# cslab-ntua/sparsex

Hardware: AMD Instinct MI355X
Metric: SpMV GFLOP/s (2*nnz/t, alpha=0.5, x/y resident in HBM) (higher is better)
Workload: dtype f64

## Files before the change

include/sparsex_hip.h:

```cpp
#ifndef SPARSEX_HIP_H
#define SPARSEX_HIP_H

#include <sparsex/sparsex.h>
#include <stdint.h>

#ifdef __cplusplus
extern "C" {
#endif

spx_error_t spx_hip_matvec_mult(spx_value_t alpha, const spx_matrix_t *A,
                                const spx_value_t *x_dev, spx_value_t *y_dev,
                                void *stream);
spx_error_t spx_hip_matvec_kernel(spx_value_t alpha, const spx_matrix_t *A,
                                  const spx_value_t *x_dev, spx_value_t beta,
                                  spx_value_t *y_dev, void *stream);

spx_error_t spx_hip_matmat_kernel(spx_value_t alpha, const spx_matrix_t *A, size_t nvec,
                                  const spx_value_t *X_dev, size_t ldx, spx_value_t beta,
                                  spx_value_t *Y_dev, size_t ldy, void *stream);
int spx_hip_matmat_group(const spx_matrix_t *A);

typedef struct spx_hip_vec spx_hip_vec_t;

void spx_hip_vec_touch(const spx_vector_t *v);
// ... 48 lines not shown
spx_hip_transport_t *spx_hip_transport_rccl(const void *id, int rank, int world);
void spx_hip_transport_destroy(spx_hip_transport_t *t);
int spx_hip_transport_rccl_ranks(const spx_hip_transport_t *t);

spx_error_t spx_hip_mat_dist_attach(spx_matrix_t *A, const spx_hip_transport_t *t);

#define SPX_DIST_OWNED_ROWS 0
#define SPX_DIST_GATHER_Y   1
#define SPX_DIST_HALO_X     2
#define SPX_DIST_OVERLAP    4
spx_error_t spx_hip_matvec_dist(spx_value_t alpha, const spx_matrix_t *A,
                                const spx_value_t *x_dev, spx_value_t beta,
                                spx_value_t *y_dev, int flags, void *stream);

typedef struct {
    int32_t rank, world;
    const spx_index_t *row_lo, *row_hi;
    int64_t n_send;
    const spx_index_t *send_rows;
    const size_t *send_off, *send_cnt;
    int64_t n_recv;
    const size_t *recv_off, *recv_cnt;
    int64_t n_fix_rows;
    const spx_index_t *fix_rows;
    const uint32_t *fix_ptr, *fix_pos;
    int32_t any_exchange;
} spx_hip_dist_plan_t;
spx_error_t spx_hip_mat_dist_plan(const spx_matrix_t *A, spx_hip_dist_plan_t *plan);

#define SPX_DIST_REORDER_RCM        1
#define SPX_DIST_REORDER_RCM_OWNER  2
#define SPX_DIST_PATTERN_SYMMETRIC  1
spx_error_t spx_hip_dist_reorder(const spx_index_t *rowptr, const spx_index_t *colind, spx_index_t nrows,
                                 int indexing , int world,
                                 int mode, int flags, spx_index_t *perm);

typedef struct {
    int64_t n_recv;
    const spx_index_t *recv_cols;
    const size_t *recv_off, *recv_cnt;
    int64_t n_send;
    const spx_index_t *send_rows;
    const size_t *send_off, *send_cnt;
} spx_hip_dist_halo_t;
spx_error_t spx_hip_mat_dist_halo(const spx_matrix_t *A, spx_hip_dist_halo_t *halo);

spx_error_t spx_hip_matvec_parts(spx_value_t alpha, const spx_matrix_t *A, const spx_value_t *x_dev,
                                 spx_value_t beta, spx_value_t *y_dev, int parts, void *stream, int *launched);

int spx_hip_mat_dist_rounds(const spx_matrix_t *A);
int spx_hip_mat_dist_parts(const spx_matrix_t *A);
spx_error_t spx_hip_mat_dist_round(const spx_matrix_t *A, int round, const size_t **send_off, const size_t **send_cnt,
                                   const size_t **recv_off, const size_t **recv_cnt);

typedef struct {
    int64_t nnz;
    int64_t nnz_stored;
    int64_t n_unit_elems;
    int64_t n_delta_elems;
    int64_t n_units;
    int64_t n_rowblocks;
    int64_t n_shared_rows;
    int64_t value_bytes;
    int64_t index_bytes;
    int32_t nr_partitions;
    int32_t first_partition, last_partition;
    int32_t row_lo, row_hi;
    int32_t symmetric;
    int32_t on_device;
    int32_t device;
    int32_t waves;
    int32_t sym_tiles;
    double  tune_seconds;
    double  emit_seconds;
    int32_t wave_tiles;
    int32_t sym_segments;
    int32_t quad;
    int32_t col_slices;
    int32_t unit_windows;
    int32_t unit_window_lds;
    int64_t unit_window_elems;
    int64_t unit_window_staged;
    int32_t sym_pipeline;
    int32_t reserved0;
    int64_t sym_pipeline_elems;
} spx_hip_info_t;

spx_error_t spx_hip_mat_info(const spx_matrix_t *A, spx_hip_info_t *info);

typedef struct {
    const uint32_t *tab;
    const uint32_t *xdescs;
    const void *passes;
    size_t n_rowblocks, n_descs, n_passes;
    size_t rowblocks_with_windows, rowblocks_with_units;
    uint64_t staged_doubles;
    uint64_t unit_elems, unit_elems_lds;
    uint32_t lds_doubles;
} spx_hip_xw_plan_t;
spx_error_t spx_hip_mat_unit_windows(spx_matrix_t *A, uint32_t budget, uint32_t gap, spx_hip_xw_plan_t *plan);

typedef struct {
    const void *passes;
    const uint32_t *n_sx;
    size_t n_rowblocks, n_passes;
    size_t rowblocks_with_sx;
    uint64_t sym_elems, sx_elems;
    uint64_t sym_passes, sx_passes;
} spx_hip_sx_plan_t;
spx_error_t spx_hip_mat_sym_pipeline(spx_matrix_t *A, spx_hip_sx_plan_t *plan);
#define SPX_HIP_ABI_VERSION 5
spx_error_t spx_hip_mat_info_sized(const spx_matrix_t *A, void *info, size_t size);
int spx_hip_abi_version(void);

int spx_hip_mat_host_parts(const spx_matrix_t *A);
int spx_hip_mat_host_order(const spx_matrix_t *A, int32_t *order, int cap);
int64_t spx_hip_mat_x_pieces(spx_matrix_t *A, size_t piece, uint64_t *mask, uint32_t *row0, uint32_t *n_rows, size_t cap);

typedef struct {
    const spx_value_t *values;
    const uint8_t *ctl;
    int64_t ctl_size;
    spx_index_t nnz, ncols, nrows, row_start;
    int32_t row_jumps;
    int32_t full_colind;
    long id_map[64];
    const spx_index_t *rows_info;
    const spx_value_t *dvalues;
} spx_csx_export_t;

spx_error_t spx_hip_mat_export_csx(const spx_matrix_t *A, int part,
                                   spx_csx_export_t *out);

typedef struct {
    int32_t type, delta, size, row, col;
} spx_unit_record_t;

int64_t spx_hip_mat_export_units(const spx_matrix_t *A, int part,
                                 spx_unit_record_t *recs, int64_t cap);

const char *spx_hip_mat_tune_log(const spx_matrix_t *A);

void spx_hip_xform(int from, int to, spx_index_t *row, spx_index_t *col,
                   spx_index_t nr_rows, spx_index_t nr_cols);

void spx_hip_options_reset(void);

#ifdef __cplusplus
}
#endif

#endif
```

sparsex_amd/api.py:

```python
import ctypes as C
import os

import numpy as np

SPX_SUCCESS = 0
SPX_FAILURE = -1
SPX_MAT_REORDER = 42
SPX_VEC_AS_IS = 43
SPX_VEC_TUNE = 44
SPX_INDEX_ZERO_BASED = 45
SPX_INDEX_ONE_BASED = 46

_HERE = os.path.dirname(os.path.abspath(__file__))


def lib_path():
    return os.environ.get("SPX_LIB_PATH") or os.path.join(_HERE, "lib", "libsparsex.so")


class SpxError(RuntimeError):
    pass


class VectorStruct(C.Structure):
    _fields_ = [("elements", C.POINTER(C.c_double)), ("size", C.c_size_t),
                ("alloc_type", C.c_int), ("vec_mode", C.c_int)]


class HipInfo(C.Structure):
    _fields_ = [("nnz", C.c_int64), ("nnz_stored", C.c_int64),
                ("n_unit_elems", C.c_int64), ("n_delta_elems", C.c_int64),
                ("n_units", C.c_int64), ("n_rowblocks", C.c_int64),
                ("n_shared_rows", C.c_int64), ("value_bytes", C.c_int64),
                ("index_bytes", C.c_int64), ("nr_partitions", C.c_int32),
                ("first_partition", C.c_int32), ("last_partition", C.c_int32),
                ("row_lo", C.c_int32), ("row_hi", C.c_int32),
                ("symmetric", C.c_int32), ("on_device", C.c_int32),
                ("device", C.c_int32), ("waves", C.c_int32), ("sym_tiles", C.c_int32),
                ("tune_seconds", C.c_double),
                ("emit_seconds", C.c_double), ("wave_tiles", C.c_int32), ("sym_segments", C.c_int32),
                ("quad", C.c_int32), ("col_slices", C.c_int32),
                ("unit_windows", C.c_int32), ("unit_window_lds", C.c_int32),
                ("unit_window_elems", C.c_int64), ("unit_window_staged", C.c_int64),
                ("sym_pipeline", C.c_int32), ("reserved0", C.c_int32), ("sym_pipeline_elems", C.c_int64)]


class SxPlan(C.Structure):
    _fields_ = [("passes", C.c_void_p), ("n_sx", C.POINTER(C.c_uint32)), ("n_rowblocks", C.c_size_t),
                ("n_passes", C.c_size_t), ("rowblocks_with_sx", C.c_size_t), ("sym_elems", C.c_uint64),
                ("sx_elems", C.c_uint64), ("sym_passes", C.c_uint64), ("sx_passes", C.c_uint64)]


class XwPlan(C.Structure):
    _fields_ = [("tab", C.POINTER(C.c_uint32)), ("xdescs", C.POINTER(C.c_uint32)), ("passes", C.c_void_p),
                ("n_rowblocks", C.c_size_t), ("n_descs", C.c_size_t), ("n_passes", C.c_size_t),
                ("rowblocks_with_windows", C.c_size_t), ("rowblocks_with_units", C.c_size_t),
                ("staged_doubles", C.c_uint64), ("unit_elems", C.c_uint64), ("unit_elems_lds", C.c_uint64),
                ("lds_doubles", C.c_uint32)]


class CsxExport(C.Structure):
    _fields_ = [("values", C.POINTER(C.c_double)), ("ctl", C.POINTER(C.c_uint8)),
                ("ctl_size", C.c_int64), ("nnz", C.c_int), ("ncols", C.c_int),
                ("nrows", C.c_int), ("row_start", C.c_int),
                ("row_jumps", C.c_int32), ("full_colind", C.c_int32),
                ("id_map", C.c_long * 64), ("rows_info", C.POINTER(C.c_int)),
                ("dvalues", C.POINTER(C.c_double))]


class UnitRecord(C.Structure):
    _fields_ = [("type", C.c_int32), ("delta", C.c_int32), ("size", C.c_int32),
                ("row", C.c_int32), ("col", C.c_int32)]


_lib = None


def lib():
    global _lib
    if _lib is not None:
        return _lib
    path = lib_path()
    if not os.path.exists(path):
        raise SpxError(
            "libsparsex.so is not built (%s); run `make lib` or "
            "__graft_entry__.build() -- there is no fallback path" % path)
    L = C.CDLL(path, mode=C.RTLD_GLOBAL)
    vp, i, d = C.c_void_p, C.c_int, C.c_double
    L.spx_input_load_csr.restype = vp
    L.spx_input_load_mmf.restype = vp
    L.spx_input_load_mmf.argtypes = [C.c_char_p]
    L.spx_input_destroy.argtypes = [vp]
    L.spx_mat_tune.restype = vp
    L.spx_mat_destroy.argtypes = [vp]
    L.spx_mat_get_nrows.argtypes = [vp]
    L.spx_mat_get_ncols.argtypes = [vp]
    L.spx_mat_get_nnz.argtypes = [vp]
    L.spx_mat_get_partition.restype = vp
    L.spx_mat_get_partition.argtypes = [vp]
    L.spx_partition_get_rs.restype = C.POINTER(C.c_int)
    L.spx_partition_get_rs.argtypes = [vp]
    L.spx_partition_get_re.restype = C.POINTER(C.c_int)
    L.spx_partition_get_re.argtypes = [vp]
    L.spx_partition_destroy.argtypes = [vp]
    L.spx_option_set.argtypes = [C.c_char_p, C.c_char_p]
    L.spx_option_set.restype = None
    L.spx_hip_options_reset.restype = None
    L.spx_vec_create_from_buff.restype = C.POINTER(VectorStruct)
    L.spx_vec_create_from_buff.argtypes = [C.POINTER(C.c_double), vp, C.c_size_t, vp,
                                           C.c_uint]
    L.spx_vec_destroy.argtypes = [C.POINTER(VectorStruct)]
    L.spx_vec_destroy.restype = None
    L.spx_matvec_mult.argtypes = [d, vp, C.POINTER(VectorStruct), C.POINTER(VectorStruct)]
    L.spx_matvec_kernel.argtypes = [d, vp, C.POINTER(VectorStruct), d,
                                    C.POINTER(VectorStruct)]
    L.spx_hip_matvec_mult.argtypes = [d, vp, vp, vp, vp]
    L.spx_hip_matvec_kernel.argtypes = [d, vp, vp, d, vp, vp]
    L.spx_hip_mat_info.argtypes = [vp, C.POINTER(HipInfo)]
    L.spx_hip_mat_export_csx.argtypes = [vp, i, C.POINTER(CsxExport)]
    L.spx_hip_mat_export_units.restype = C.c_int64
    L.spx_hip_mat_export_units.argtypes = [vp, i, C.POINTER(UnitRecord), C.c_int64]
    L.spx_hip_mat_tune_log.restype = C.c_char_p
    L.spx_hip_mat_tune_log.argtypes = [vp]
    L.spx_hip_vec_create.restype = vp
    L.spx_hip_vec_create.argtypes = [C.c_size_t]
    L.spx_hip_vec_destroy.argtypes = [vp]
    L.spx_hip_vec_data.restype = vp
# ... 90 lines not shown
        try:
            if beta is None:
                rc = L.spx_matvec_mult(alpha, self.handle, xv, yv)
            else:
                rc = L.spx_matvec_kernel(alpha, self.handle, xv, beta, yv)
        finally:
            L.spx_vec_destroy(xv)
            L.spx_vec_destroy(yv)
        if rc != SPX_SUCCESS:
            raise SpxError("spx_matvec failed (see stderr)")
        return y

    def partition(self):
        L = lib()
        p = L.spx_mat_get_partition(self.handle)
        n = self.info().nr_partitions
        rs = [L.spx_partition_get_rs(p)[i] for i in range(n)]
        re = [L.spx_partition_get_re(p)[i] for i in range(n)]
        L.spx_partition_destroy(p)
        return rs, re

    def hip_matvec_mult(self, alpha, x_ptr, y_ptr, stream=0):
        rc = lib().spx_hip_matvec_mult(alpha, self.handle, x_ptr, y_ptr, stream)
        if rc != SPX_SUCCESS:
            raise SpxError("spx_hip_matvec_mult failed (see stderr)")

    def hip_matvec_kernel(self, alpha, x_ptr, beta, y_ptr, stream=0):
        rc = lib().spx_hip_matvec_kernel(alpha, self.handle, x_ptr, beta, y_ptr, stream)
        if rc != SPX_SUCCESS:
            raise SpxError("spx_hip_matvec_kernel failed (see stderr)")

    def hip_matmat_kernel(self, alpha, x_ptr, ldx, nvec, beta, y_ptr, ldy, stream=0):
        L = lib()
        L.spx_hip_matmat_kernel.restype = C.c_int
        L.spx_hip_matmat_kernel.argtypes = [C.c_double, C.c_void_p, C.c_size_t, C.c_void_p, C.c_size_t,
                                            C.c_double, C.c_void_p, C.c_size_t, C.c_void_p]
        rc = L.spx_hip_matmat_kernel(alpha, self.handle, nvec, x_ptr, ldx, beta, y_ptr, ldy, stream)
        if rc != SPX_SUCCESS:
            raise SpxError("spx_hip_matmat_kernel failed (see stderr)")

    def matmat_group(self):
        L = lib()
        L.spx_hip_matmat_group.restype = C.c_int
        L.spx_hip_matmat_group.argtypes = [C.c_void_p]
        return int(L.spx_hip_matmat_group(C.c_void_p(self.handle)))

    def matmat(self, alpha, X, beta, Y, stream=None):
        import torch
        pairs = (("X", X, self.ncols), ("Y", Y, self.nrows))
        for name, t, n in pairs:
            if not isinstance(t, torch.Tensor):
                raise ValueError("%s must be a torch tensor" % name)
            if t.dtype != torch.float64:
                raise ValueError("%s must be float64, not %s" % (name, t.dtype))
            if t.dim() != 2 or t.shape[1] != n:
                raise ValueError("%s must have the shape (nvec, %d), not %s" % (name, n, tuple(t.shape)))
            if t.shape[0] > 0 and t.shape[1] > 1 and t.stride(1) != 1:
                raise ValueError("%s needs stride(1) == 1, not %d" % (name, t.stride(1)))
            if t.shape[0] > 1 and t.stride(0) < n:
                raise ValueError("%s: stride(0) %d is below the vector length %d" % (name, t.stride(0), n))
        if X.shape[0] != Y.shape[0]:
            raise ValueError("X holds %d vectors, Y %d" % (X.shape[0], Y.shape[0]))
        for name, t, n in pairs:
            if t.device.type != "cuda":
                raise ValueError("%s must live on the matrix' HIP device, not on %s" % (name, t.device))
        if X.device != Y.device:
            raise ValueError("X and Y live on different devices (%s, %s)" % (X.device, Y.device))
        inf = self.info()
        if inf.on_device and X.device.index != inf.device:
            raise ValueError("the matrix lives on cuda:%d, the tensors on %s" % (inf.device, X.device))
        nvec = int(X.shape[0])
        ldx = max(int(X.stride(0)), self.ncols) if nvec > 1 else max(self.ncols, 1)
        ldy = max(int(Y.stride(0)), self.nrows) if nvec > 1 else max(self.nrows, 1)
        st = stream if stream is not None else torch.cuda.current_stream(Y.device)
        self.hip_matmat_kernel(alpha, X.data_ptr(), ldx, nvec, beta, Y.data_ptr(), ldy, st.cuda_stream)
        return Y

    def info(self):
        inf = HipInfo()
        if lib().spx_hip_mat_info(self.handle, C.byref(inf)) != SPX_SUCCESS:
            raise SpxError("spx_hip_mat_info failed")
        return inf

    def unit_windows(self, budget=4096, gap=16):
        pl = XwPlan()
        L = lib()
        L.spx_hip_mat_unit_windows.argtypes = [C.c_void_p, C.c_uint32, C.c_uint32, C.POINTER(XwPlan)]
        if L.spx_hip_mat_unit_windows(self.handle, budget, gap, C.byref(pl)) != SPX_SUCCESS:
            raise SpxError("spx_hip_mat_unit_windows failed")
        out = {k: getattr(pl, k) for k in ("n_rowblocks", "n_descs", "n_passes", "rowblocks_with_windows",
                                           "rowblocks_with_units", "staged_doubles", "unit_elems",
                                           "unit_elems_lds", "lds_doubles")}
        out["tab"] = np.ctypeslib.as_array(pl.tab, shape=(pl.n_rowblocks * 32,)).reshape(-1, 16, 2).copy() \
            if pl.n_rowblocks else np.zeros((0, 16, 2), np.uint32)
        out["xdescs"] = np.ctypeslib.as_array(pl.xdescs, shape=(pl.n_descs * 2,)).reshape(-1, 2).copy() \
            if pl.n_descs else np.zeros((0, 2), np.uint32)
        raw = C.string_at(pl.passes, pl.n_passes * 24) if pl.n_passes else b""
        out["passes"] = np.frombuffer(raw, dtype=np.uint8).reshape(-1, 24).copy()
        return out

    def sym_pipeline(self):
        import numpy as np
        pl = SxPlan()
        L = lib()
        L.spx_hip_mat_sym_pipeline.argtypes = [C.c_void_p, C.POINTER(SxPlan)]
        if L.spx_hip_mat_sym_pipeline(self.handle, C.byref(pl)) != SPX_SUCCESS:
            raise SpxError("spx_hip_mat_sym_pipeline failed")
        passes = np.ctypeslib.as_array(C.cast(pl.passes, C.POINTER(C.c_uint32)), shape=(pl.n_passes, 6)).copy() \
            if pl.n_passes else np.zeros((0, 6), np.uint32)
        n_sx = np.ctypeslib.as_array(pl.n_sx, shape=(pl.n_rowblocks,)).copy() if pl.n_rowblocks else np.zeros(0, np.uint32)
        return passes, n_sx, {k: int(getattr(pl, k)) for k in ("rowblocks_with_sx", "sym_elems", "sx_elems",
                                                                "sym_passes", "sx_passes")}

    def host_parts(self):
        L = lib()
        L.spx_hip_mat_host_parts.restype = C.c_int
        return int(L.spx_hip_mat_host_parts(C.c_void_p(self.handle)))

    def host_order(self):
        L = lib()
        L.spx_hip_mat_host_order.restype = C.c_int
        L.spx_hip_mat_host_order.argtypes = [C.c_void_p, C.POINTER(C.c_int32), C.c_int]
        buf = (C.c_int32 * 64)()
        k = L.spx_hip_mat_host_order(C.c_void_p(self.handle), buf, 64)
        return [int(buf[i]) for i in range(min(k, 64))]

    def x_pieces(self, piece):
        import numpy as np
        L = lib()
        L.spx_hip_mat_x_pieces.restype = C.c_int64
        L.spx_hip_mat_x_pieces.argtypes = [C.c_void_p, C.c_size_t, C.c_void_p, C.c_void_p, C.c_void_p, C.c_size_t]
        n = L.spx_hip_mat_x_pieces(C.c_void_p(self.handle), piece, None, None, None, 0)
        if n < 0:
            raise SpxError("spx_hip_mat_x_pieces failed")
        m, r0, nr = np.zeros(n, np.uint64), np.zeros(n, np.uint32), np.zeros(n, np.uint32)
        if n and L.spx_hip_mat_x_pieces(C.c_void_p(self.handle), piece, m.ctypes.data, r0.ctypes.data, nr.ctypes.data, n) != n:
            raise SpxError("spx_hip_mat_x_pieces failed")
        return m, r0, nr

    def export_csx(self, part=0):
        ex = CsxExport()
        if lib().spx_hip_mat_export_csx(self.handle, part, C.byref(ex)) != SPX_SUCCESS:
            raise SpxError("spx_hip_mat_export_csx failed")
        out = {
            "values": np.ctypeslib.as_array(ex.values, shape=(max(ex.nnz, 0),)).copy()
            if ex.nnz else np.zeros(0),
            "ctl": np.ctypeslib.as_array(ex.ctl, shape=(ex.ctl_size,)).copy()
            if ex.ctl_size else np.zeros(0, dtype=np.uint8),
            "nnz": ex.nnz, "ncols": ex.ncols, "nrows": ex.nrows,
            "row_start": ex.row_start, "row_jumps": int(ex.row_jumps),
            "full_colind": int(ex.full_colind),
            "id_map": [int(v) for v in ex.id_map],
            "rows_info": np.ctypeslib.as_array(ex.rows_info, shape=(ex.nrows, 3)).copy()
            if ex.nrows else np.zeros((0, 3), dtype=np.int32),
            "dvalues": (np.ctypeslib.as_array(ex.dvalues, shape=(ex.nrows,)).copy()
                        if bool(ex.dvalues) and ex.nrows else None),
        }
        return out

    def export_units(self, part=0):
        L = lib()
        n = L.spx_hip_mat_export_units(self.handle, part, None, 0)
        if n < 0:
            raise SpxError("spx_hip_mat_export_units failed")
        recs = (UnitRecord * max(n, 1))()
        L.spx_hip_mat_export_units(self.handle, part, recs, n)
# ... 441 lines not shown
```

sparsex_amd/csrc/api.cpp:

```cpp
#include <sparsex/sparsex.h>
#include <sparsex_hip.h>

#include "config.hpp"
#include "csx_emit.hpp"
#include "device.hpp"
#include "dist.hpp"
#include "encoder.hpp"
#include "gpu_emit.hpp"
#include "input.hpp"
#include "reorder.hpp"
#include "stream_index.hpp"
#include "threads.hpp"

#include <chrono>
#include <cmath>
#include <cstdarg>
#include <cstdint>
#include <cstring>
#include <functional>
#include <memory>
#include <mutex>
#include <atomic>
#include <sstream>
#include <thread>
// ... 495 lines not shown
            if (use_segs) A->sym_atomic = true;
            if (use_segs) gp.skip_empty = true;
            emit_pieces(fulls, &tiles, use_segs ? &segs : nullptr);
            {
                struct Gone {
                    std::vector<Partition> fulls;
                    std::vector<SymSegVec> segs;
                    std::vector<std::vector<SymTile>> tiles;
                };
                Gone *g = new Gone();
                g->fulls.swap(fulls);
                g->segs.swap(segs);
                g->tiles.swap(tiles);
                release_after_upload = [g] {
                    parallel_for(g->fulls.size(), host_threads(), [&](size_t i) {
                        g->fulls[i] = Partition();
                        if (i < g->segs.size()) SymSegVec().swap(g->segs[i]);
                        if (i < g->tiles.size()) std::vector<SymTile>().swap(g->tiles[i]);
                    });
                    delete g;
                };
            }
            for (size_t k = 0; k < thin.size(); ++k) {
                if (k == 0 || thin[k].row != thin[k - 1].row) {
                    gs.mirror_rows.push_back((uint32_t) thin[k].row);
                    gs.mirror_ptr.push_back((uint32_t) k);
                }
                gs.mirror_col.push_back((uint32_t) thin[k].col);
                gs.mirror_val.push_back(thin[k].val);
            }
            gs.mirror_ptr.push_back((uint32_t) thin.size());
            gs.nnz_stored += thin.size();
            gs.n_delta_elems += thin.size();
        } else {
            Partition full;
            for (size_t i = 0; i < nown; ++i) append_sym_expanded(A->parts[i], full, gp.sym_remine);
            if (gs.sym_fused) full.nr_rows = (size_t) A->nrows;
            emit_gpu(full, gp, gs, hw);
        }
    } else if (A->col_phases <= 1) {
        emit_pieces(A->parts, nullptr);
    } else {
        const size_t K = A->col_phases;
        GpuEmitParams keep = gp;
        gp.max_rows = std::max<size_t>(gp.max_rows, SPX_MAX_WIDE_ROWS);
        for (size_t k = 0; k < K; ++k) {
            const idx_t c_lo = (idx_t)((int64_t) A->ncols * (int64_t) k / (int64_t) K) + 1;
            const idx_t c_hi = (idx_t)((int64_t) A->ncols * (int64_t)(k + 1) / (int64_t) K) + 1;
            std::vector<Partition> sub(nown);
            parallel_for(nown, hw, [&](size_t i) {
                const Partition &p = A->parts[i];
                Partition &q = sub[i];
                q.nr_rows = p.nr_rows; q.nr_cols = p.nr_cols; q.type = p.type; q.row_start = p.row_start;
                q.pool = p.pool;
                for (size_t e = 0; e < p.elems_size; ++e)
                    if (p.elems[e].col >= c_lo && p.elems[e].col < c_hi) {
                        q.elems.push_back(p.elems[e]);
                        q.nnz += p.elems[e].size;
                    }
                q.elems_size = q.elems.size();
            });
            gp.skip_empty = k > 0 || A->col_concurrent;
            const size_t rb0 = gs.rbs.size();
            emit_pieces(sub, nullptr);
            if (k > 0 && gs.rbs.size() > rb0) gs.rbs[rb0].flags |= SPX_RB_PHASE_START;
            if (A->col_concurrent && gs.rbs.size() == rb0) throw FatalError("column phases: an empty slice");
        }
        if (A->col_concurrent)
            for (SpxRowBlock &rb : gs.rbs) rb.flags |= SPX_RB_ACCUM;
        gp = keep;
        if (!gs.shared.empty()) throw FatalError("column phases: the matrix holds rows that are split over row-blocks");
    }
    const double t_emit1 = now_sec();
    A->conflict_rows.clear();
    if (sym && !gs.sym_fused) stream_touched_rows(gs, A->own_lo, A->conflict_rows);
    A->halo_cols.clear();
    if (A->own_lo > 0 || A->own_hi < A->nrows) stream_read_cols(gs, A->own_lo, A->own_hi, (size_t) A->ncols, A->halo_cols);
    A->first_block_row = A->own_lo;
    for (const SpxRowBlock &rb : gs.rbs) A->first_block_row = std::min<idx_t>(A->first_block_row, (idx_t) rb.row0);
    finalize_stream(gs, (size_t) A->nrows);
    if (sym) mark_private_rowblocks(gs, (size_t) A->nrows, A->own_lo, A->own_hi);
    std::vector<std::pair<uint32_t, uint32_t>>().swap(gs.direct_cols);
    gs.waves = (uint32_t) A->waves;
    gs.band_order = Config::instance().get_bool("spx.gpu.band_order");
    gs.arena = Config::instance().get_bool("spx.gpu.arena");
    gs.xw_budget = (A->unit_windows != 0 && !A->deterministic && !sym) ? (A->rb_joined ? std::max(A->xw_budget, JOINED_XW_BUDGET) : A->xw_budget) : 0u;
    gs.xw_gap = A->xw_gap;
    gs.xw_on = A->xw_on;
    gs.sx_plan = sym && A->sym_pipeline != 0 && !A->deterministic && A->wave_tiles != 1;
    gs.sx_on = A->sx_on;
    gs.sym_atomic = A->sym_atomic && !A->deterministic;
    gs.deterministic = A->deterministic;
    gs.wave_tiles = A->deterministic || A->wave_tiles == 1;
    A->nnz_stored = gs.nnz_stored;
    A->n_unit_elems = gs.n_unit_elems;
    A->n_delta_elems = gs.n_delta_elems;
    A->n_units = gs.n_units;
    A->value_bytes = gs.values.size() * sizeof(val_t);
    A->index_bytes = gs.index_bytes();
    A->n_rowblocks = gs.rbs.size();
    A->n_shared = gs.shared.size();
    A->has_tiles = stream_has_tiles(gs);
    A->has_symtiles = stream_has_pass(gs, SPX_PASS_SYMTILE);
    if (A->dev) {
        device_free(A->dev);
        A->dev = nullptr;
    }
    const double t_emit2 = now_sec();
    if (!A->host_only) {
        A->dev = device_upload(gs, (size_t) A->nrows, (size_t) A->ncols, sym, A->own_lo, A->own_hi,
                               A->device_ordinal);
        log_msg(LOG_INFO, "descriptor stream: emitted in %.2f s, finalized in %.2f s, uploaded in %.2f s (%zu row-blocks)\n",
                t_emit1 - t_emit0, t_emit2 - t_emit1, now_sec() - t_emit2, gs.rbs.size());
        if (A->dist && sym) {
            device_set_init_rows(A->dev, (size_t) dist_first_init_row(*A));
        }
        keep_index(A, std::move(gs));
    } else {
        A->host_stream.reset(new GpuStream(std::move(gs)));
    }
    if (release_after_upload) {
        std::function<void()> f;
        f.swap(release_after_upload);
        A->release_wait();
        A->release_later(std::move(f));
    }
}

static void autotune_launch(spx_matrix_t *A, bool tune_waves, bool tune_spill, bool tune_wave_tiles, bool tune_xw)
{
    A->release_wait();
    const double t_est = device_time_spmv(A->dev, 2, 3);
    const int N = (int) std::min(100.0, std::max(8.0, 0.02 / std::max(t_est, 1e-7)));
    const int W = std::max(2, N / 10);
    auto best_time = [&]() {
        A->release_wait();
        double best = device_time_spmv(A->dev, W, N);
        for (int rep = 0; rep < 3; ++rep) best = std::min(best, device_time_spmv(A->dev, 0, N));
        return best;
    };
    auto time_xw = [&](bool &xw) {
        if (!tune_xw || !device_has_xw(A->dev) || A->wave_tiles == 1) {
            xw = device_get_xw(A->dev);
            return best_time();
        }
        device_set_xw(A->dev, false);
        const double t0 = best_time();
        device_set_xw(A->dev, true);
        const double t1 = best_time();
        xw = t1 < 0.985 * t0;
        device_set_xw(A->dev, xw);
        return std::min(t0, xw ? t1 : t0);
    };
    if (!tune_waves) {
        if (tune_wave_tiles && !device_has_tiles(A->dev) && !(A->unit_windows == 1 && device_has_xw(A->dev))) {
            auto t_of = [&](bool on) {
                device_set_wave_tiles(A->dev, on);
                return best_time();
            };
            const double t0 = t_of(false), t1 = t_of(true);
            A->wave_tiles = t1 < 0.985 * t0 ? 1 : 0;
            device_set_wave_tiles(A->dev, A->wave_tiles == 1);
        }
        if (tune_xw && device_has_xw(A->dev) && A->wave_tiles != 1) {
            bool xw = false;
            (void) time_xw(xw);
            A->xw_on = xw;
// ... 234 lines not shown
    A->emit_params.target_elems = (size_t) std::max<long>(64, rbe);
    A->emit_params.max_rows = (size_t) std::min<long>(SPX_MAX_WIDE_ROWS, std::max<long>(1, cfg.get_long("spx.gpu.rowblock_rows")));
    A->emit_params.sym_remine = cfg.get_bool("spx.gpu.sym_remine");
    A->emit_params.sym_once = cfg.get_bool("spx.gpu.sym_once");
    A->emit_params.recut_linear = cfg.get_bool("spx.gpu.recut_linear");
    A->emit_params.keep_units = cfg.get_bool("spx.gpu.keep_units");
    A->emit_params.inline_desc = cfg.get_bool("spx.gpu.inline_desc");
    A->emit_params.sym_pure_passes = cfg.get_bool("spx.gpu.sym_pure_passes");
    A->emit_params.x_window = cfg.get_bool("spx.gpu.x_window");
    {
        const std::string m = cfg.get_str("spx.gpu.sym_segments");
        if (m != "auto" && m != "true" && m != "false") {
            log_msg(LOG_ERR, "spx.gpu.sym_segments: true, false or auto\n");
            throw FatalError("bad spx.gpu.sym_segments");
        }
        A->emit_params.sym_segments = m == "auto" ? -1 : (m == "true" ? 1 : 0);
        const long wide = cfg.get_long("spx.gpu.sym_wide_rows");
        if (wide < 1 || wide > SPX_MAX_WIDE_ROWS) {
            log_msg(LOG_ERR, "spx.gpu.sym_wide_rows: 1 .. %d\n", SPX_MAX_WIDE_ROWS);
            throw FatalError("bad spx.gpu.sym_wide_rows");
        }
        A->emit_params.wide_rows = (size_t) wide;
        const long mr = cfg.get_long("spx.gpu.sym_segment_min");
        if (mr < 2 || mr > 8) {
            log_msg(LOG_ERR, "spx.gpu.sym_segment_min: 2 .. 8\n");
            throw FatalError("bad spx.gpu.sym_segment_min");
        }
        A->emit_params.sym_min_run = (size_t) mr;
        const long xr = cfg.get_long("spx.gpu.sym_segment_max");
        if (xr < mr || xr > SPX_MAX_SEG_WIDTH) {
            log_msg(LOG_ERR, "spx.gpu.sym_segment_max: spx.gpu.sym_segment_min .. %d\n", SPX_MAX_SEG_WIDTH);
            throw FatalError("bad spx.gpu.sym_segment_max");
        }
        A->emit_params.sym_max_run = (size_t) xr;
    }
    A->emit_params.stack_segments = cfg.get_bool("spx.gpu.stack_segments");
    {
        idx_t lo = nown ? A->bounds[first].row_start : 0;
        idx_t hi = nown ? A->bounds[last - 1].row_start + A->bounds[last - 1].nr_rows : 0;
        if (last == P) hi = rows_end;
        A->own_lo = lo;
        A->own_hi = hi;
    }
    A->waves = (int) cfg.get_long("spx.gpu.waves");
    const bool autotune = A->waves == 0;
    if (autotune) A->waves = 4;
    const std::string spill_mode = cfg.get_str("spx.gpu.sym_spill");
    if (spill_mode != "auto" && spill_mode != "lists" && spill_mode != "atomic") {
        log_msg(LOG_ERR, "spx.gpu.sym_spill: lists, atomic or auto\n");
        throw FatalError("bad spx.gpu.sym_spill");
    }
    A->deterministic = cfg.get_bool("spx.gpu.deterministic");
    A->sym_atomic = spill_mode == "atomic" && !A->deterministic;
    A->spill_mode = spill_mode == "lists" ? 0 : (spill_mode == "atomic" ? 1 : -1);
    const std::string wt_mode = cfg.get_str("spx.gpu.wave_tiles");
    if (wt_mode != "auto" && wt_mode != "true" && wt_mode != "false") {
        log_msg(LOG_ERR, "spx.gpu.wave_tiles: true, false or auto\n");
        throw FatalError("bad spx.gpu.wave_tiles");
    }
    A->wave_tiles = wt_mode == "true" ? 1 : 0;
    const std::string xw_mode = cfg.get_str("spx.gpu.unit_windows");
    if (xw_mode != "auto" && xw_mode != "true" && xw_mode != "false") {
        log_msg(LOG_ERR, "spx.gpu.unit_windows: true, false or auto\n");
        throw FatalError("bad spx.gpu.unit_windows");
    }
    {
        const long xb = cfg.get_long("spx.gpu.unit_window_doubles"), xg = cfg.get_long("spx.gpu.unit_window_gap");
        if (xb < 0 || xb > 16384 || xg < 0 || xg > 255) {
            log_msg(LOG_ERR, "spx.gpu.unit_window_doubles: 0 .. 16384, spx.gpu.unit_window_gap: 0 .. 255\n");
            throw FatalError("bad spx.gpu.unit_window_doubles / spx.gpu.unit_window_gap");
        }
        A->xw_budget = (uint32_t) xb;
        A->xw_gap = (uint32_t) xg;
    }
    A->unit_windows = xw_mode == "auto" ? -1 : (xw_mode == "true" ? 1 : 0);
    A->xw_on = xw_mode == "true";
    const std::string sx_mode = cfg.get_str("spx.gpu.sym_pipeline");
    if (sx_mode != "auto" && sx_mode != "true" && sx_mode != "false") {
        log_msg(LOG_ERR, "spx.gpu.sym_pipeline: true, false or auto\n");
        throw FatalError("bad spx.gpu.sym_pipeline");
    }
    A->sym_pipeline = sx_mode == "auto" ? -1 : (sx_mode == "true" ? 1 : 0);
    A->sx_on = sx_mode == "true";
    const std::string ph_mode = cfg.get_str("spx.gpu.col_phases");
    const bool ph_conc = ph_mode.size() == 2 && ph_mode[0] == 'c';
    long ph_fixed = ph_mode == "auto" ? 0 : strtol(ph_mode.c_str() + (ph_conc ? 1 : 0), nullptr, 10);
    if (ph_mode != "auto" && (ph_fixed < 1 || ph_fixed > 8 || (ph_conc && ph_fixed != 2 && ph_fixed != 4 && ph_fixed != 8))) {
        log_msg(LOG_ERR, "spx.gpu.col_phases: 1 .. 8 (launched in turn), c2 | c4 | c8 (one launch, a group of XCDs each) or auto\n");
        throw FatalError("bad spx.gpu.col_phases");
    }
    A->col_phases = (!sym && ph_fixed > 1) ? (size_t) ph_fixed : 1;
    A->col_concurrent = A->col_phases > 1 && ph_conc && !A->deterministic;
    if (A->col_phases > 1 && ph_conc && !A->col_concurrent) A->col_phases = 1;
    try {
        emit_and_upload(A.get());
    } catch (const FatalError &) {
        if (A->col_phases <= 1) throw;
        A->col_phases = 1;
        emit_and_upload(A.get());
    }
    const bool tune_spill = spill_mode == "auto" && !A->deterministic && !A->has_symsegs;
    const bool tune_wt = wt_mode == "auto" && !A->deterministic && !A->has_symsegs;
    const bool tune_xw = xw_mode == "auto" && !A->deterministic && !sym;
    const double t_auto = now_sec();
    if (A->dev && A->nnz_stored >= 100000 && (autotune || tune_spill || tune_wt || tune_xw))
        autotune_launch(A.get(), autotune, tune_spill, tune_wt, tune_xw);
    if (A->dev && sym && A->sym_pipeline == -1 && device_has_sx(A->dev)) {
        A->release_wait();
        const double t_est = device_time_spmv(A->dev, 2, 3);
        const int N = (int) std::min(100.0, std::max(8.0, 0.02 / std::max(t_est, 1e-7)));
        auto best_of = [&](bool on) {
            device_set_sx(A->dev, on);
            double best = device_time_spmv(A->dev, std::max(2, N / 10), N);
            for (int rep = 0; rep < 3; ++rep) best = std::min(best, device_time_spmv(A->dev, 0, N));
            return best;
        };
        const double t0 = best_of(false), t1 = best_of(true);
        A->sx_on = t1 < 0.985 * t0;
        device_set_sx(A->dev, A->sx_on);
        log_msg(LOG_INFO, "read-once pipeline: %s (%.2f us per SpMV with, %.2f without)\n", A->sx_on ? "on" : "off", 1e6 * t1, 1e6 * t0);
    }
    const double t_auto_end = now_sec();
    if (A->dev && !sym && ph_mode == "auto" && A->n_shared == 0 && A->nnz_stored >= 100000 &&
        2 * A->n_delta_elems >= A->nnz_stored && (size_t) A->ncols * sizeof(val_t) >= ((size_t) 6 << 20)) {
        auto best_of = [&]() {
            double best = device_time_spmv(A->dev, 10, 100);
            for (int rep = 0; rep < 3; ++rep) best = std::min(best, device_time_spmv(A->dev, 0, 100));
            return best;
        };
        const double t_plain = best_of();
        size_t K = 1;
        double t_ph = t_plain;
        if (!A->deterministic) {
            for (size_t k : {(size_t) 2, (size_t) 4}) {
                if ((size_t) A->ncols * sizeof(val_t) < k * ((size_t) 3 << 19)) break;
                try {
                    A->col_phases = k;
                    A->col_concurrent = true;
                    emit_and_upload(A.get());
                    const double t = best_of();
                    if (t < 0.97 * t_ph) {
                        t_ph = t;
                        K = k;
                    }
                } catch (const FatalError &) {
                    break;
                }
            }
        }
        if (A->col_phases != K || !A->col_concurrent) {
            A->col_phases = K;
            A->col_concurrent = K > 1;
            emit_and_upload(A.get());
        }
        log_msg(LOG_INFO, "column slices: %zu on XCD groups %.2f us, plain %.2f us per SpMV\n", K, 1e6 * t_ph, 1e6 * t_plain);
    }

    if (!cfg.get_bool("spx.rt.keep_encoded")) {
        std::vector<Partition> *old = new std::vector<Partition>();
        old->swap(A->parts);
        A->release_later([old] {
            parallel_for(old->size(), host_threads(), [&](size_t i) { (*old)[i] = Partition(); });
            delete old;
        });
    }
    log_msg(LOG_INFO, "launch parameters measured in %.2f s\n", t_auto_end - t_auto);
    A->emit_seconds = now_sec() - t1;
    return A.release();
}

spx_matrix_t *spx_mat_tune(spx_input_t *in, ...)
try {
    if (!in) {
        SETERROR_1(SPX_ERR_ARG_INVALID, "invalid input matrix");
        return SPX_INVALID_MAT;
    }
    va_list ap;
    va_start(ap, in);
    spx_option_t option = va_arg(ap, spx_option_t);
    va_end(ap);
    std::vector<idx_t> perm;
    if (option == SPX_MAT_REORDER && Config::instance().get_long("spx.rt.global_rows") > 0) {
        SETWARNING(SPX_WARN_REORDER);
        option = 0;
    }
    int re_mode = SPX_DIST_REORDER_RCM;
    size_t re_world = 1;
    {
        const std::string dr = Config::instance().get_str("spx.rt.dist_reorder");
        const long world = Config::instance().get_long("spx.rt.gpu_world");
        if (dr != "none" && dr != "rcm" && dr != "rcm_owner") {
            SETERROR_1(SPX_ERR_ARG_INVALID, "spx.rt.dist_reorder: none, rcm or rcm_owner");
            return SPX_INVALID_MAT;
        }
        if (dr != "none" && world > 1 && Config::instance().get_long("spx.rt.global_rows") <= 0) {
            option = SPX_MAT_REORDER;
            re_mode = dr == "rcm_owner" ? SPX_DIST_REORDER_RCM_OWNER : SPX_DIST_REORDER_RCM;
            re_world = (size_t) world;
        }
    }
    if (option == SPX_MAT_REORDER) {
        MatrixInput *re = nullptr;
        try {
// ... 441 lines not shown
                get_vec(f, gs->cidx) && get_vec(f, gs->segrows) && get_vec(f, gs->shared) &&
                get_vec(f, gs->dvalues) && get_vec(f, gs->values) && get_vec(f, gs->fix_ptr) &&
                get_vec(f, gs->fix_idx) && get_vec(f, gs->slot_group_col) && get_vec(f, gs->mirror_rows) &&
                get_vec(f, gs->mirror_ptr) && get_vec(f, gs->mirror_col) && get_vec(f, gs->mirror_val);
    std::vector<int32_t> perm;
    good = good && get_vec(f, perm);
    std::unique_ptr<matrix> A(new matrix);
    if (good && h.n_encoded) {
        good = h.n_encoded == h.last_part - h.first_part && h.n_encoded <= (1u << 20);
        if (good) {
            A->parts.resize(h.n_encoded);
            if (h.symmetric) A->diag.resize(h.n_encoded);
        }
        std::vector<val_t> nodiag;
        for (uint32_t i = 0; good && i < h.n_encoded; ++i)
            good = get_partition(f, A->parts[i], h.symmetric ? A->diag[i] : nodiag);
    }
    fclose(f);
    std::string why = "not a tuned-matrix file of this build";
    if (good) {
        good = h.nrows >= 0 && h.ncols >= 0 && bnd.size() == 3 * h.nr_partitions &&
               h.first_part <= h.last_part && h.last_part <= h.nr_partitions &&
               (perm.empty() || perm.size() == (size_t) h.nrows) && h.own_lo >= 0 &&
               h.own_lo <= h.own_hi && h.own_hi <= h.nrows &&
               (!h.symmetric || gs->dvalues.size() == (size_t) h.nrows);
        for (int32_t v : perm) good = good && v >= 0 && v < h.nrows;
    }
    if (good) {
        gs->n_carry = h.n_carry;
        gs->sym_fused = (h.pad & 1u) != 0;
        gs->pass_stride = h.pad >> 1;
        gs->n_spill = h.n_spill;
        gs->lds_doubles = h.lds_doubles;
        gs->waves = h.waves;
        gs->sym_atomic = h.sym_atomic != 0;
        gs->deterministic = (h.pad3 & 1u) != 0;
        gs->wave_tiles = (h.pad3 & 2u) != 0;
        gs->xw_on = (h.pad3 & 4u) != 0;
        gs->sx_on = (h.pad3 & 8u) != 0;
        gs->sx_plan = gs->sx_on;
        gs->xw_gap = gs->xw_on ? ((h.pad3 >> 8) & 255u) : 16u;
        gs->xw_budget = gs->xw_on ? (h.pad3 >> 16) : 0u;
        gs->nnz_stored = h.nnz_stored; gs->n_unit_elems = h.n_unit_elems;
        gs->n_delta_elems = h.n_delta_elems; gs->n_units = h.n_units;
        good = stream_checksum(*gs) == h.checksum;
        if (!good) why = "tuned-matrix file is damaged (checksum of the index arrays)";
        else good = stream_validate(*gs, (size_t) h.nrows, (size_t) h.ncols, gs->values.size(), why);
    }
    if (!good) {
        SETERROR_1(SPX_ERR_FILE, why.c_str());
        return SPX_INVALID_MAT;
    }
    A->nrows = h.nrows; A->ncols = h.ncols; A->nnz = h.nnz; A->symmetric = h.symmetric;
    A->permutation = SPX_INVALID_PERM;
    if (!perm.empty()) {
        A->permutation = (spx_perm_t *) malloc(perm.size() * sizeof(spx_perm_t));
        std::copy(perm.begin(), perm.end(), A->permutation);
    }
    A->nr_partitions = h.nr_partitions; A->first_part = h.first_part; A->last_part = h.last_part;
    for (size_t i = 0; i < h.nr_partitions; ++i)
        A->bounds.push_back(PartBounds{bnd[3 * i], bnd[3 * i + 1], (size_t) bnd[3 * i + 2]});
    A->full_colind = false;
    A->dev = nullptr;
    A->waves = (h.waves == 2 || h.waves == 8) ? (int) h.waves : 4;
    A->own_lo = h.own_lo; A->own_hi = h.own_hi;
    A->nnz_stored = h.nnz_stored; A->n_unit_elems = h.n_unit_elems;
    A->n_delta_elems = h.n_delta_elems; A->n_units = h.n_units;
    A->value_bytes = gs->values.size() * sizeof(val_t);
    A->index_bytes = gs->index_bytes();
    A->n_rowblocks = gs->rbs.size();
    A->n_shared = gs->shared.size();
    A->has_tiles = stream_has_tiles(*gs);
    A->has_symtiles = stream_has_pass(*gs, SPX_PASS_SYMTILE);
    A->has_symsegs = stream_has_symsegs(*gs);
    A->sym_atomic = gs->sym_atomic;
    A->deterministic = gs->deterministic;
    A->wave_tiles = gs->wave_tiles ? 1 : 0;
    A->xw_on = gs->xw_on;
    A->unit_windows = gs->xw_on ? 1 : 0;
    A->sx_on = gs->sx_on;
    A->sym_pipeline = gs->sx_on ? 1 : 0;
    A->xw_budget = gs->xw_budget;
    A->xw_gap = gs->xw_gap;
    {
        size_t slices = 1;
        for (size_t i = 1; i < gs->rbs.size(); ++i) slices += (gs->rbs[i].flags & SPX_RB_PHASE_START) ? 1 : 0;
        A->col_phases = slices;
        A->col_concurrent = slices > 1 && !gs->rbs.empty() && (gs->rbs[0].flags & SPX_RB_ACCUM);
    }
    A->tune_seconds = 0.0;
    A->auto_rb = false;
    const double t0 = now_sec();
    Config &cfg = Config::instance();
    A->host_only = cfg.get_bool("spx.rt.host_only");
    A->device_ordinal = (int) cfg.get_long("spx.rt.device");
    A->full_colind = cfg.get_bool("spx.matrix.full_colind");
    if (A->symmetric && !gs->sym_fused) stream_touched_rows(*gs, A->own_lo, A->conflict_rows);
    if (A->own_lo > 0 || A->own_hi < A->nrows) stream_read_cols(*gs, A->own_lo, A->own_hi, (size_t) A->ncols, A->halo_cols);
    A->first_block_row = A->own_lo;
    for (const SpxRowBlock &rb : gs->rbs) A->first_block_row = std::min<idx_t>(A->first_block_row, (idx_t) rb.row0);
    try {
        if (!A->host_only) {
            A->dev = device_upload(*gs, (size_t) A->nrows, (size_t) A->ncols, A->symmetric != 0,
                                   A->own_lo, A->own_hi, A->device_ordinal);
            keep_index(A.get(), std::move(*gs));
        } else {
            A->host_stream = std::move(gs);
        }
    } catch (const FatalError &) {
        SETERROR_0(SPX_ERR_TUNED_MAT);
        return SPX_INVALID_MAT;
    }
    A->emit_seconds = now_sec() - t0;
    return A.release();
} SPX_C_BOUNDARY(return SPX_INVALID_MAT;)

spx_index_t spx_mat_get_nrows(const spx_matrix_t *A)
try {
    if (!A) { SETERROR_1(SPX_ERR_ARG_INVALID, "invalid matrix handle"); return SPX_FAILURE; }
    return A->nrows;
} SPX_C_BOUNDARY(return 0;)

spx_index_t spx_mat_get_ncols(const spx_matrix_t *A)
try {
    if (!A) { SETERROR_1(SPX_ERR_ARG_INVALID, "invalid matrix handle"); return SPX_FAILURE; }
    return A->ncols;
} SPX_C_BOUNDARY(return 0;)

spx_index_t spx_mat_get_nnz(const spx_matrix_t *A)
try {
    if (!A) { SETERROR_1(SPX_ERR_ARG_INVALID, "invalid matrix handle"); return SPX_FAILURE; }
    return A->nnz;
} SPX_C_BOUNDARY(return 0;)

static spx_partition_t *part_alloc(size_t n)
{
    spx_partition_t *p = (spx_partition_t *) malloc(sizeof(spx_partition_t));
    p->nr_partitions = n;
    p->parts = NULL;
    p->nodes = NULL;
    p->affinity = NULL;
    p->row_start = (spx_index_t *) malloc(sizeof(spx_index_t) * (n ? n : 1));
    p->row_end = (spx_index_t *) malloc(sizeof(spx_index_t) * (n ? n : 1));
    return p;
}

spx_partition_t *spx_mat_get_partition(const spx_matrix_t *A)
try {
    if (!A) {
        SETERROR_1(SPX_ERR_ARG_INVALID, "invalid matrix handle");
        return SPX_INVALID_PART;
    }
    spx_partition_t *p = part_alloc(A->nr_partitions);
    for (size_t i = 0; i < A->nr_partitions; ++i) {
        p->row_start[i] = A->bounds[i].row_start;
        p->row_end[i] = A->bounds[i].row_start + A->bounds[i].nr_rows;
    }
    return p;
} SPX_C_BOUNDARY(return SPX_INVALID_PART;)

spx_index_t *spx_partition_get_rs(const spx_partition_t *p)
try {
    if (!p) { SETERROR_1(SPX_ERR_ARG_INVALID, "invalid partition handle"); return NULL; }
    return p->row_start;
} SPX_C_BOUNDARY(return nullptr;)

// ... 274 lines not shown
        return SPX_FAILURE;
    }
    const uintptr_t x0 = (uintptr_t) X_dev, x1 = x0 + ((nvec - 1) * ldx + nc) * sizeof(double);
    const uintptr_t y0 = (uintptr_t) Y_dev, y1 = y0 + ((nvec - 1) * ldy + nr) * sizeof(double);
    if (x0 < y1 && y0 < x1) {
        SETERROR_1(SPX_ERR_ARG_INVALID, "blocks X and Y overlap");
        return SPX_FAILURE;
    }
    try {
        device_spmm(A->dev, alpha, X_dev, ldx, nvec, beta, Y_dev, ldy, stream);
    } catch (const FatalError &e) {
        SETERROR_1(SPX_ERR_TUNED_MAT, e.what.c_str());
        return SPX_FAILURE;
    }
    return SPX_SUCCESS;
} SPX_C_BOUNDARY(return SPX_FAILURE;)

int spx_hip_matmat_group(const spx_matrix_t *A)
try {
    return A && A->dev ? device_mv_group(A->dev) : -1;
} SPX_C_BOUNDARY(return -1;)


int spx_hip_abi_version(void) { return SPX_HIP_ABI_VERSION; }

int spx_hip_mat_host_parts(const spx_matrix_t *A)
try {
    return A && A->dev ? device_host_parts(A->dev) : 0;
} SPX_C_BOUNDARY(return 0;)

int spx_hip_mat_host_order(const spx_matrix_t *A, int32_t *order, int cap)
try {
    return A && A->dev && (order || cap <= 0) ? device_host_order(A->dev, order, cap < 0 ? 0 : cap) : 0;
} SPX_C_BOUNDARY(return 0;)

spx_error_t spx_hip_mat_unit_windows(spx_matrix_t *A, uint32_t budget, uint32_t gap, spx_hip_xw_plan_t *out)
try {
    if (!A || !out) { SETERROR_1(SPX_ERR_ARG_INVALID, "invalid argument"); return SPX_FAILURE; }
    const GpuStream *s = A->host_stream ? A->host_stream.get() : A->index.get();
    if (!s) { SETERROR_1(SPX_ERR_TUNED_MAT, "matrix holds no descriptor stream"); return SPX_FAILURE; }
    std::lock_guard<std::mutex> lk(A->mtx);
    try {
        std::unique_ptr<XwPlan> plan(new XwPlan);
        plan_unit_xwindows(*s, (size_t) A->ncols, A->symmetric ? 0u : budget, gap, *plan, host_threads());
        A->xw_inspect = std::move(plan);
    } catch (const FatalError &e) {
        SETERROR_1(SPX_ERR_TUNED_MAT, e.what.c_str());
        return SPX_FAILURE;
    } catch (const std::exception &e) {
        SETERROR_1(SPX_ERR_MEM_ALLOC, e.what());
        return SPX_FAILURE;
    }
    const XwPlan &p = *A->xw_inspect;
    memset(out, 0, sizeof(*out));
    out->tab = reinterpret_cast<const uint32_t *>(p.tab.data());
    out->xdescs = reinterpret_cast<const uint32_t *>(p.xdescs.data());
    out->passes = p.passes.data();
    out->n_rowblocks = s->rbs.size();
    out->n_descs = p.xdescs.size();
    out->n_passes = p.passes.size();
    out->rowblocks_with_windows = p.n_rb_windows;
    out->rowblocks_with_units = p.n_rb_units;
    out->staged_doubles = p.staged_doubles;
    out->unit_elems = p.unit_elems;
    out->unit_elems_lds = p.unit_elems_lds;
    out->lds_doubles = p.lds_doubles;
    return SPX_SUCCESS;
} SPX_C_BOUNDARY(return SPX_FAILURE;)

int64_t spx_hip_mat_x_pieces(spx_matrix_t *A, size_t piece, uint64_t *mask, uint32_t *row0, uint32_t *n_rows, size_t cap)
try {
    if (!A || !piece) { SETERROR_1(SPX_ERR_ARG_INVALID, "invalid argument"); return -1; }
    const GpuStream *s = A->host_stream ? A->host_stream.get() : A->index.get();
    if (!s) { SETERROR_1(SPX_ERR_TUNED_MAT, "matrix holds no descriptor stream"); return -1; }
    std::lock_guard<std::mutex> lk(A->mtx);
    std::vector<uint64_t> m;
    stream_rowblock_xpieces(*s, (size_t) A->ncols, piece, m, host_threads());
    for (size_t i = 0; i < m.size() && i < cap; ++i) {
        if (mask) mask[i] = m[i];
        if (row0) row0[i] = s->rbs[i].row0;
        if (n_rows) n_rows[i] = s->rbs[i].n_rows;
    }
    return (int64_t) m.size();
} SPX_C_BOUNDARY(return -1;)

spx_error_t spx_hip_mat_sym_pipeline(spx_matrix_t *A, spx_hip_sx_plan_t *out)
try {
    if (!A || !out) { SETERROR_1(SPX_ERR_ARG_INVALID, "invalid argument"); return SPX_FAILURE; }
    const GpuStream *s = A->host_stream ? A->host_stream.get() : A->index.get();
    if (!s) { SETERROR_1(SPX_ERR_TUNED_MAT, "matrix holds no descriptor stream"); return SPX_FAILURE; }
    std::lock_guard<std::mutex> lk(A->mtx);
    try {
        std::unique_ptr<SxPlan> plan(new SxPlan);
        plan_sym_pipeline(*s, *plan, host_threads());
        A->sx_inspect = std::move(plan);
    } catch (const FatalError &e) {
        SETERROR_1(SPX_ERR_TUNED_MAT, e.what.c_str());
        return SPX_FAILURE;
    } catch (const std::exception &e) {
        SETERROR_1(SPX_ERR_MEM_ALLOC, e.what());
        return SPX_FAILURE;
    }
    const SxPlan &p = *A->sx_inspect;
    memset(out, 0, sizeof(*out));
    out->passes = p.passes.data();
    out->n_sx = p.n_sx.data();
    out->n_rowblocks = s->rbs.size();
    out->n_passes = p.passes.size();
    out->rowblocks_with_sx = p.n_rb_sx;
    out->sym_elems = p.sym_elems;
    out->sx_elems = p.sx_elems;
    out->sym_passes = p.sym_passes;
    out->sx_passes = p.sx_passes;
    return SPX_SUCCESS;
} SPX_C_BOUNDARY(return SPX_FAILURE;)

spx_error_t spx_hip_mat_info_sized(const spx_matrix_t *A, void *info, size_t size)
try {
    spx_hip_info_t full;
    if (!info || spx_hip_mat_info(A, &full) != SPX_SUCCESS) {
        if (!info) SETERROR_1(SPX_ERR_ARG_INVALID, "invalid argument");
        return SPX_FAILURE;
    }
    memcpy(info, &full, std::min(size, sizeof(full)));
    return SPX_SUCCESS;
} SPX_C_BOUNDARY(return SPX_FAILURE;)

spx_error_t spx_hip_mat_info(const spx_matrix_t *A, spx_hip_info_t *info)
try {
    if (!A || !info) { SETERROR_1(SPX_ERR_ARG_INVALID, "invalid argument"); return SPX_FAILURE; }
    memset(info, 0, sizeof(*info));
    info->nnz = A->nnz;
    info->nnz_stored = (int64_t) A->nnz_stored;
    info->n_unit_elems = (int64_t) A->n_unit_elems;
    info->n_delta_elems = (int64_t) A->n_delta_elems;
    info->n_units = (int64_t) A->n_units;
    info->n_rowblocks = (int64_t) A->n_rowblocks;
    info->n_shared_rows = (int64_t) A->n_shared;
    info->value_bytes = (int64_t) A->value_bytes;
    info->index_bytes = (int64_t) A->index_bytes;
    info->nr_partitions = (int32_t) A->nr_partitions;
    info->first_partition = (int32_t) A->first_part;
    info->last_partition = (int32_t) A->last_part;
    info->row_lo = A->own_lo;
    info->row_hi = A->own_hi;
    info->symmetric = A->symmetric;
    info->on_device = A->dev ? 1 : 0;
    if (A->dev) {
        DeviceMatrixInfo di;
        device_info(A->dev, di);
        info->device = di.device;
    }
    info->waves = A->dev ? device_get_waves(A->dev) : A->waves;
    info->sym_tiles = A->has_tiles ? ((A->dev ? device_get_sym_atomic(A->dev) : A->sym_atomic) ? 2 : 1) : 0;
    info->wave_tiles = A->dev ? (device_get_wave_tiles(A->dev) ? 1 : 0) : (A->wave_tiles == 1 || A->deterministic ? 1 : 0);
    info->sym_segments = A->has_symsegs ? (A->has_symtiles ? 1 : 2) : 0;
    info->col_slices = A->col_phases > 1 ? (A->col_concurrent ? (int32_t) A->col_phases : -(int32_t) A->col_phases) : 1;
    info->quad = 0;
    if (A->dev && device_has_xw(A->dev)) {
        uint64_t el = 0, ue = 0, st = 0;
        uint32_t lds = 0;
        device_xw_info(A->dev, el, ue, st, lds);
        info->unit_windows = device_get_xw(A->dev) ? 1 : 0;
        info->unit_window_lds = (int32_t) lds;
        info->unit_window_elems = (int64_t) el;
        info->unit_window_staged = (int64_t) st;
    }
    if (A->dev && device_has_sx(A->dev)) {
        uint64_t esx = 0, esym = 0;
        size_t nrb = 0;
        device_sx_info(A->dev, esx, esym, nrb);
        info->sym_pipeline = device_get_sx(A->dev) ? 1 : 0;
        info->sym_pipeline_elems = (int64_t) esx;
    }
    info->tune_seconds = A->tune_seconds;
    info->emit_seconds = A->emit_seconds;
    return SPX_SUCCESS;
} SPX_C_BOUNDARY(return SPX_FAILURE;)

static bool owned_part(const spx_matrix_t *A, int part)
{
    return part >= (int) A->first_part && part < (int) A->last_part &&
           (size_t)(part - (int) A->first_part) < A->parts.size();
}

spx_error_t spx_hip_mat_export_csx(const spx_matrix_t *A_, int part, spx_csx_export_t *out)
try {
    spx_matrix_t *A = const_cast<spx_matrix_t *>(A_);
    if (!A || !out) { SETERROR_1(SPX_ERR_ARG_INVALID, "invalid argument"); return SPX_FAILURE; }
    if (!owned_part(A, part)) {
        SETERROR_1(SPX_ERR_ARG_INVALID, "partition not held by this process "
                   "(or dropped: spx.rt.keep_encoded=false)");
        return SPX_FAILURE;
    }
    std::lock_guard<std::mutex> lk(A->mtx);
    size_t li = (size_t) part - A->first_part;
    if (A->exported.size() < A->parts.size()) {
        A->exported.resize(A->parts.size());
        A->exported_rows_info.resize(A->parts.size());
    }
    if (!A->exported[li]) {
        std::unique_ptr<CsxStream> s(new CsxStream);
        emit_csx(A->parts[li], A->full_colind, A->symmetric != 0, *s);
        if (A->symmetric) {
            s->dvalues = A->diag[li];
            s->dvalues.resize((size_t) s->nrows, 0.0);
        }
        std::vector<spx_index_t> &ri = A->exported_rows_info[li];
        ri.resize(s->rows_info.size() * 3);
        for (size_t i = 0; i < s->rows_info.size(); ++i) {
            ri[3 * i] = s->rows_info[i].rowptr;
            ri[3 * i + 1] = s->rows_info[i].valptr;
            ri[3 * i + 2] = s->rows_info[i].span;
        }
        A->exported[li] = std::move(s);
    }
    const CsxStream &s = *A->exported[li];
    memset(out, 0, sizeof(*out));
    out->values = s.values.data();
    out->ctl = s.ctl.data();
    out->ctl_size = (int64_t) s.ctl.size();
    out->nnz = s.nnz;
    out->ncols = s.ncols;
    out->nrows = s.nrows;
    out->row_start = s.row_start;
    out->row_jumps = s.row_jumps;
    out->full_colind = s.full_colind;
    for (int i = 0; i < 64; ++i) out->id_map[i] = s.id_map[i];
    out->rows_info = A->exported_rows_info[li].data();
    out->dvalues = A->symmetric ? s.dvalues.data() : NULL;
    return SPX_SUCCESS;
} SPX_C_BOUNDARY(return SPX_FAILURE;)

int64_t spx_hip_mat_export_units(const spx_matrix_t *A, int part, spx_unit_record_t *recs,
                                 int64_t cap)
try {
    if (!A || !owned_part(A, part)) {
        SETERROR_1(SPX_ERR_ARG_INVALID, "partition not held by this process");
        return -1;
    }
    const Partition &p = A->parts[(size_t) part - A->first_part];
    for (size_t i = 0; i < p.elems_size && (int64_t) i < cap && recs; ++i) {
        const Elem &e = p.elems[i];
        recs[i].type = e.type;
        recs[i].delta = (int32_t) e.delta;
        recs[i].size = e.size;
        recs[i].row = e.row;
        recs[i].col = e.col;
    }
    return (int64_t) p.elems_size;
} SPX_C_BOUNDARY(return 0;)

const char *spx_hip_mat_tune_log(const spx_matrix_t *A)
try {
    return A ? A->log.c_str() : "";
} SPX_C_BOUNDARY(return nullptr;)

// ... 252 lines not shown
```

sparsex_amd/csrc/config.cpp:

```cpp
#include "config.hpp"

#include <cstdlib>
#include <regex>
#include <sstream>

namespace spx {

Config &Config::instance()
{
    static Config c;
    return c;
}

Config::Config() { reset_defaults(); }

void Config::reset_defaults()
{
    props_.clear();
    props_["spx.rt.nr_threads"] = "1";
    props_["spx.rt.cpu_affinity"] = "0";
    props_["spx.preproc.heuristic"] = "ratio";
    props_["spx.preproc.xform"] = "all";
    props_["spx.preproc.sampling"] = "portion";
    props_["spx.preproc.sampling.nr_samples"] = "48";
    props_["spx.preproc.sampling.portion"] = "0.01";
    props_["spx.preproc.sampling.window_size"] = "0";
    props_["spx.matrix.symmetric"] = "false";
    props_["spx.matrix.split_blocks"] = "true";
    props_["spx.matrix.full_colind"] = "false";
    props_["spx.matrix.min_unit_size"] = "4";
    props_["spx.matrix.max_unit_size"] = "255";
    props_["spx.matrix.min_coverage"] = "0.1";
    props_["spx.matrix.onedim_blocks"] = "false";
    props_["spx.rt.host_only"] = "false";
    props_["spx.rt.gpu_rank"] = "0";
    props_["spx.rt.gpu_world"] = "1";
    props_["spx.rt.device"] = "-1";
    props_["spx.vec.register"] = "auto";
    props_["spx.vec.device"] = "false";
    props_["spx.rt.host_parts"] = "0";
    props_["spx.rt.dist_chunks"] = "4";
    props_["spx.rt.dist_reorder"] = "none";
    props_["spx.rt.row_offset"] = "0";
    props_["spx.rt.global_rows"] = "0";
    props_["spx.rt.keep_encoded"] = "true";
    props_["spx.gpu.rowblock_elems"] = "0";
    props_["spx.gpu.rowblock_rows"] = "512";
    props_["spx.gpu.stack_segments"] = "true";
    props_["spx.gpu.waves"] = "0";
    props_["spx.gpu.inline_desc"] = "true";
    props_["spx.gpu.arena"] = "false";
    props_["spx.gpu.band_order"] = "false";
    props_["spx.gpu.col_phases"] = "auto";
    props_["spx.gpu.keep_units"] = "true";
    props_["spx.gpu.recut_linear"] = "true";
    props_["spx.gpu.sym_once"] = "true";
    props_["spx.gpu.deterministic"] = "false";
    props_["spx.gpu.wave_tiles"] = "auto";
    props_["spx.gpu.x_window"] = "true";
    props_["spx.gpu.sym_segments"] = "auto";
    props_["spx.gpu.sym_segment_min"] = "2";
    props_["spx.gpu.sym_segment_max"] = "8";
    props_["spx.gpu.sym_wide_rows"] = "1024";
    props_["spx.gpu.sym_spill"] = "auto";
    props_["spx.gpu.sym_remine"] = "true";
    props_["spx.gpu.sym_pure_passes"] = "true";
    props_["spx.gpu.sym_pipeline"] = "auto";
    props_["spx.gpu.unit_windows"] = "auto";
    props_["spx.gpu.unit_window_doubles"] = "3072";
    props_["spx.gpu.unit_window_gap"] = "16";
}

bool Config::set(const std::string &key, const std::string &value)
{
    auto it = props_.find(key);
    if (it == props_.end()) {
        log_msg(LOG_WARN, "mnemonic \"%s\" not found\n", key.c_str());
        return false;
    }
    if (key == "spx.preproc.heuristic" && value != "ratio" && value != "cost") {
        log_msg(LOG_ERR, "invalid value \"%s\" while setting property "
                "\"spx.preproc.heuristic\"\n", value.c_str());
        throw FatalError("invalid heuristic");
    }
    if (key == "spx.preproc.sampling" && value != "none" && value != "window" &&
        value != "portion") {
        log_msg(LOG_ERR, "invalid value \"%s\" while setting property "
                "\"spx.preproc.sampling\"\n", value.c_str());
        throw FatalError("invalid sampling method");
    }
    it->second = value;
    return true;
}

void Config::load_from_env()
{
    const char *s;
    if ((s = getenv("SYMMETRIC"))) set("spx.matrix.symmetric", s);
    if ((s = getenv("CPU_AFFINITY"))) set("spx.rt.cpu_affinity", s);
    if ((s = getenv("NUM_THREADS"))) set("spx.rt.nr_threads", s);
    if ((s = getenv("XFORM_CONF"))) set("spx.preproc.xform", s);
    if ((s = getenv("WINDOW_SIZE"))) {
        set("spx.preproc.sampling", "window");
        set("spx.preproc.sampling.window_size", s);
    }
    if ((s = getenv("SAMPLES"))) set("spx.preproc.sampling.nr_samples", s);
    if ((s = getenv("SAMPLING_PORTION"))) {
        set("spx.preproc.sampling", "portion");
        set("spx.preproc.sampling.portion", s);
    }
    if ((s = getenv("SAMPLING"))) set("spx.preproc.sampling", s);
    if ((s = getenv("SPX_VEC_DEVICE"))) set("spx.vec.device", s);
}

std::string Config::get_str(const std::string &key) const
{
    auto it = props_.find(key);
    if (it == props_.end()) {
        log_msg(LOG_ERR, "property \"%s\" not found\n", key.c_str());
        throw FatalError("unknown property");
    }
    return it->second;
}

long Config::get_long(const std::string &key) const
{
    std::string v = get_str(key);
    char *end = nullptr;
    long r = strtol(v.c_str(), &end, 10);
    if (end == v.c_str() || *end != '\0') {
        log_msg(LOG_ERR, "invalid value \"%s\" while setting property \"%s\"\n",
                v.c_str(), key.c_str());
        throw FatalError("bad integer property");
    }
    return r;
// ... 80 lines not shown
```

sparsex_amd/csrc/device.hpp:

```cpp
#pragma once

#include "gpu_emit.hpp"

#include <functional>
#include <string>
#include <vector>

namespace spx {

struct DeviceMatrix;

int device_count();
DeviceMatrix *device_upload(const GpuStream &s, size_t nrows, size_t ncols,
                            bool symmetric, idx_t own_row_lo, idx_t own_row_hi,
                            int device);
void device_free(DeviceMatrix *m);

void device_spmv(DeviceMatrix *m, double alpha, const double *d_x, double beta,
                 double *d_y, void *stream);

void device_spmm(DeviceMatrix *m, double alpha, const double *d_X, size_t ldx, size_t nvec, double beta,
                 double *d_Y, size_t ldy, void *stream);
int device_mv_group(const DeviceMatrix *m);

size_t device_plan_chunks(DeviceMatrix *m, size_t K, std::vector<size_t> &row_bounds, int slot = 0);
void device_spmv_chunk(DeviceMatrix *m, size_t k, double alpha, const double *d_x, double beta,
                       double *d_y, void *stream, int slot = 0, int position = -1);

void device_spmv_host(DeviceMatrix *m, double alpha, const double *h_x, bool x_pinned,
                      double beta, double *h_y, bool y_pinned,
                      const std::function<void(double *, void *)> &after = nullptr,
                      uint64_t x_version = 0);

bool device_stream_is_capturing(void *stream);

void *device_host_alloc(size_t bytes);
void device_host_free(void *p);
size_t device_host_parts_min_bytes();
int device_host_register(void *p, size_t bytes);
void device_host_unregister(void *p);

void device_set_init_rows(DeviceMatrix *m, size_t first_row);

void device_set_sym_atomic(DeviceMatrix *m, bool on);
bool device_get_sym_atomic(const DeviceMatrix *m);
bool device_has_spill(const DeviceMatrix *m);

void device_set_deterministic(DeviceMatrix *m, bool on);
bool device_get_deterministic(const DeviceMatrix *m);
void device_set_wave_tiles(DeviceMatrix *m, bool on);
bool device_get_wave_tiles(const DeviceMatrix *m);
bool device_has_tiles(const DeviceMatrix *m);

void device_set_waves(DeviceMatrix *m, int waves);
int device_get_waves(const DeviceMatrix *m);

bool device_has_xw(const DeviceMatrix *m);
int device_host_order(const DeviceMatrix *m, int32_t *order, int cap);
void device_set_host_parts(DeviceMatrix *m, size_t parts);
int device_host_parts(const DeviceMatrix *m);
void device_set_xw(DeviceMatrix *m, bool on);
bool device_get_xw(const DeviceMatrix *m);
void device_xw_info(const DeviceMatrix *m, uint64_t &elems_lds, uint64_t &unit_elems, uint64_t &staged_doubles,
                    uint32_t &lds_bytes);

bool device_has_sx(const DeviceMatrix *m);
void device_set_sx(DeviceMatrix *m, bool on);
bool device_get_sx(const DeviceMatrix *m);
void device_sx_info(const DeviceMatrix *m, uint64_t &elems_sx, uint64_t &elems_sym, size_t &rowblocks);

double device_time_spmv(DeviceMatrix *m, int warmup, int launches);

void device_download(const DeviceMatrix *m, GpuStream &s);

double device_peek(const DeviceMatrix *m, bool diagonal, size_t index);
void device_poke(DeviceMatrix *m, bool diagonal, size_t index, double value);
void device_poke_mirror(DeviceMatrix *m, size_t index, double value);

struct DeviceMatrixInfo {
    size_t n_rowblocks, n_shared_rows;
    size_t value_bytes, index_bytes;
    int device;
};
void device_info(const DeviceMatrix *m, DeviceMatrixInfo &info);

}
```

sparsex_amd/csrc/device_runtime.cpp:

```cpp
#include "device.hpp"
#include "hip_check.hpp"
#include "spmv_launch.hpp"
#include "spx_abl.hpp"
#include "stream_index.hpp"
#include "sxplan.hpp"
#include "threads.hpp"
#include "xwindows.hpp"

#include <hip/hip_runtime_api.h>

#include <algorithm>
#include <cstdio>
#include <cstdlib>
#include <cstring>
#include <string>
#include <type_traits>
#include <vector>

namespace spx {

struct DeviceMatrix {
    int device = 0;
    size_t nrows = 0, ncols = 0;
    bool symmetric = false;
    bool sym_fused = false;
    uint32_t pass_stride = 1;
    size_t own_lo = 0, own_hi = 0;
    size_t init_lo = 0;
    bool init_limited = false;
    uint32_t n_rb = 0, n_shared = 0, n_carry = 0;
    double *carry_mv = nullptr;
    uint32_t mv_rows = 0, mv_xwin = 0;
    SpxRowBlock *rbs = nullptr;
    double *values = nullptr;
    SpxUnitDesc *descs = nullptr;
    SpxPass *passes = nullptr;
    uint8_t *cidx = nullptr;
    uint16_t *segrows = nullptr;
    SpxSharedRow *shared = nullptr;
    double *carry = nullptr;
    double *dvalues = nullptr;
    bool has_tiles = false;
    int waves = 4;
    int waves_req = 4;
    uint32_t n_spill = 0, lds_doubles = SPX_MAX_RB_ROWS;
    double *spill = nullptr;
    uint32_t *fix_ptr = nullptr, *fix_idx = nullptr;
    size_t n_fix_ptr = 0, n_fix_idx = 0;
    bool sym_atomic = false;
    size_t n_private_rb = 0;
    bool use_private = false;
    size_t max_slot_groups = 0;
    std::vector<XcdSplit> xcd_split;
    std::vector<uint32_t> xcd_longest;
    bool accum = false;
    std::vector<uint32_t> launch_order;
    size_t band_stride = 0;
    bool launched_since_edit = true;
    bool has_symsegs = false;
    bool has_symtiles = false;
    bool wave_tiles = false;
    bool deterministic = false;
    uint32_t *slot_col = nullptr;
    size_t n_slot_col = 0;
    std::vector<std::pair<size_t, size_t>> private_rows;
    uint32_t n_mirror_rows = 0;
    size_t n_mirror_nnz = 0;
    uint32_t *mirror_rows = nullptr, *mirror_ptr = nullptr, *mirror_col = nullptr;
    double *mirror_val = nullptr;
    double *d_x = nullptr, *d_y = nullptr;
    double *p_x = nullptr, *p_y = nullptr;
    uint64_t x_version = 0;
    hipStream_t host_stream = nullptr;
    hipStream_t copy_stream = nullptr;
    std::vector<hipEvent_t> stage_events;
    std::vector<hipEvent_t> part_events;
    int host_parts = 0;
    bool host_x_by_need = false;
    size_t host_parts_want = 0;
    size_t value_bytes = 0, index_bytes = 0;
    size_t n_values = 0, n_descs = 0, n_passes = 0, n_cidx = 0, n_segrows = 0;
    void *arena = nullptr;
    size_t arena_bytes = 0;
    std::vector<uint64_t> rb_upto;
    std::vector<uint32_t> rb_row0;
    struct ChunkPlan {
        std::vector<XcdSplit> split;
        std::vector<uint32_t> longest;
        std::vector<size_t> bounds;
        size_t asked = 0;
        std::vector<uint32_t> order;
        std::vector<std::vector<uint32_t>> step_pieces;
        XcdSplit front;
        uint32_t front_longest = 0;
    };
    ChunkPlan chunks[3];
    SpxPass *passes_xw = nullptr;
    SpxUnitDesc *xdescs = nullptr;
    XwEntry *xw_tab = nullptr;
    uint32_t lds_doubles_xw = 0;
    uint32_t xw_budget = 0, xw_gap = 0;
    bool xw_on = false;
    uint64_t xw_elems = 0, xw_unit_elems = 0, xw_staged = 0;
    size_t xw_rowblocks = 0;
    SpxPass *passes_sx = nullptr;
    uint32_t *sx_tab = nullptr;
    bool sx_on = false;
    uint64_t sx_elems = 0, sx_sym_elems = 0;
    size_t sx_rowblocks = 0;
    std::vector<uint64_t> rb_xneed;
    size_t xneed_piece = 0;
    hipStream_t up_stream = nullptr;
};

constexpr int MV_MAX_GROUP = 8;
constexpr size_t MV_LDS_BUDGET = (size_t) 80 << 10;

constexpr size_t STAGE_PIECE = (size_t) 16 << 20;
constexpr size_t HOST_PARTS = 8;
constexpr size_t HOST_PARTS_X = 24, HOST_PARTS_X_SYM = 16;
constexpr size_t HOST_X_PIECE = (size_t) 4 << 20;
constexpr size_t HOST_PARTS_MIN_BYTES = (size_t) 32 << 20;

static size_t host_parts_min_bytes()
{
    static const size_t v = getenv("SPX_HOST_PARTS_MIN_BYTES") ? (size_t) atoll(getenv("SPX_HOST_PARTS_MIN_BYTES"))
                                                               : HOST_PARTS_MIN_BYTES;
    return v;
}

static size_t host_xpiece_doubles(size_t ncols)
{
    static const size_t env = getenv("SPX_HOST_XPIECE_BYTES") ? (size_t) atoll(getenv("SPX_HOST_XPIECE_BYTES")) / sizeof(double) : 0;
    size_t piece = env ? env : HOST_X_PIECE / sizeof(double);
    piece = std::max(piece, (ncols + 63) / 64);
    return (piece + 511) & ~(size_t) 511;
}

int device_count()
{
    int n = 0;
    if (hipGetDeviceCount(&n) != hipSuccess) return 0;
    return n;
}

struct Placement {
    struct Item { void **dst; const void *src; size_t copy_bytes, alloc_bytes; };
    std::vector<Item> items;
    template <typename T, typename A>
    void put(T **dst, const std::vector<T, A> &v, size_t slack_elems = 0)
    {
        size_t bytes = (v.size() + slack_elems) * sizeof(T);
        if (bytes == 0) bytes = sizeof(T);
        items.push_back(Item{reinterpret_cast<void **>(dst), v.data(), v.size() * sizeof(T), bytes});
    }
    static size_t piece(size_t bytes)
    {
        const size_t a = bytes >= ((size_t) 1 << 20) ? ((size_t) 2 << 20) : 256u;
        return (bytes + a - 1) / a * a;
    }
    void flush(DeviceMatrix *m, bool arena)
    {
        if (!arena) {
            for (const Item &it : items) {
                void *d = nullptr;
                HIP_CHECK(hipMalloc(&d, it.alloc_bytes));
                *it.dst = d;
                HIP_CHECK(hipMemset(d, 0, it.alloc_bytes));
                if (it.copy_bytes) HIP_CHECK(hipMemcpy(d, it.src, it.copy_bytes, hipMemcpyHostToDevice));
            }
            return;
        }
        size_t total = 0;
        for (const Item &it : items) total += piece(it.alloc_bytes);
        total = (total + ((size_t) 2 << 20) - 1) & ~(((size_t) 2 << 20) - 1);
        void *base = nullptr;
        HIP_CHECK(hipMalloc(&base, total));
        m->arena = base;
        m->arena_bytes = total;
        HIP_CHECK(hipMemset(base, 0, total));
        std::vector<size_t> order(items.size());
        for (size_t i = 0; i < order.size(); ++i) order[i] = i;
        std::stable_sort(order.begin(), order.end(), [&](size_t a, size_t b) { return items[a].alloc_bytes > items[b].alloc_bytes; });
        size_t at = 0;
        for (size_t i : order) {
            const Item &it = items[i];
            char *d = static_cast<char *>(base) + at;
            *it.dst = d;
            if (it.copy_bytes) HIP_CHECK(hipMemcpy(d, it.src, it.copy_bytes, hipMemcpyHostToDevice));
            at += piece(it.alloc_bytes);
        }
    }
};

DeviceMatrix *device_upload(const GpuStream &s, size_t nrows, size_t ncols,
                            bool symmetric, idx_t own_lo, idx_t own_hi, int device)
{
    if (device_count() <= 0) {
        log_msg(LOG_ERR, "no usable HIP device: the SpMV path of this library runs "
                "on an MI355X only (set spx.rt.host_only=true to tune without one)\n");
        throw FatalError("no HIP device");
    }
    if (device >= 0) HIP_CHECK(hipSetDevice(device));
    if (!s.pass_stride && !s.rbs.empty()) throw FatalError("descriptor stream was not finalized");
    DeviceMatrix *m = new DeviceMatrix;
    HIP_CHECK(hipGetDevice(&m->device));
    m->nrows = nrows;
    m->ncols = ncols;
    m->symmetric = symmetric;
    m->sym_fused = symmetric && s.sym_fused;
    m->pass_stride = s.pass_stride;
    m->waves = m->waves_req = (s.waves == 2 || s.waves == 8) ? (int) s.waves : 4;
    m->own_lo = (size_t) own_lo;
    m->own_hi = (size_t) own_hi;
    m->n_rb = (uint32_t) s.rbs.size();
    m->n_shared = (uint32_t) s.shared.size();
    m->n_carry = s.n_carry;
    Placement place;
    const std::vector<double> no_doubles;
    std::vector<double> dv;
    std::vector<SpxRowBlock> rbs_ordered;
    std::vector<SpxPass> passes_ordered;
    place.put(&m->cidx, s.cidx, 64);
    place.put(&m->segrows, s.segrows, 80);
    place.put(&m->shared, s.shared);
    place.put(&m->carry, no_doubles, s.n_carry ? s.n_carry : 1);
    if (symmetric) {
        dv = s.dvalues;
        dv.resize(nrows, 0.0);
        place.put(&m->dvalues, dv);
    }
    m->n_spill = s.n_spill;
    m->lds_doubles = s.lds_doubles;
    for (const SpxRowBlock &rb : s.rbs)
        for (uint32_t k = 0; k < rb.n_pass && !m->has_tiles; ++k)
            m->has_tiles = s.passes[rb.pass_off + k].kind == SPX_PASS_SYMTILE ||
                           s.passes[rb.pass_off + k].kind == SPX_PASS_SYMSEG;
    if (!m->has_tiles) {
        for (const SpxRowBlock &rb : s.rbs) {
            m->mv_rows = std::max<uint32_t>(m->mv_rows, rb.n_rows);
            m->mv_xwin = std::max<uint32_t>(m->mv_xwin, rb.xwin_len);
        }
        place.put(&m->carry_mv, no_doubles, (size_t) MV_MAX_GROUP * (s.n_carry ? s.n_carry : 1));
        spmv_mv_allow_lds(160u * 1024u);
    }
    for (const SpxRowBlock &rb : s.rbs)
        for (uint32_t k = 0; k < rb.n_pass && !m->has_symsegs; ++k)
            m->has_symsegs = s.passes[rb.pass_off + k].kind == SPX_PASS_SYMSEG;
    for (const SpxRowBlock &rb : s.rbs)
        for (uint32_t k = 0; k < rb.n_pass && !m->has_symtiles; ++k)
            m->has_symtiles = s.passes[rb.pass_off + k].kind == SPX_PASS_SYMTILE;
    if (s.n_spill) {
        place.put(&m->spill, no_doubles, s.n_spill);
        place.put(&m->fix_ptr, s.fix_ptr);
        place.put(&m->fix_idx, s.fix_idx);
        m->n_fix_ptr = s.fix_ptr.size();
        m->n_fix_idx = s.fix_idx.size();
        place.put(&m->slot_col, s.slot_group_col);
        m->n_slot_col = s.slot_group_col.size();
    }
    if (!s.mirror_rows.empty()) {
        m->n_mirror_rows = (uint32_t) s.mirror_rows.size();
        m->n_mirror_nnz = s.mirror_col.size();
        place.put(&m->mirror_rows, s.mirror_rows);
        place.put(&m->mirror_ptr, s.mirror_ptr);
        place.put(&m->mirror_col, s.mirror_col);
        place.put(&m->mirror_val, s.mirror_val);
    }
    m->sym_atomic = (s.sym_atomic || m->has_symsegs) && m->has_tiles;
    {
        std::vector<std::pair<size_t, size_t>> pr;
        for (const SpxRowBlock &rb : s.rbs)
            if (rb.flags & SPX_RB_PRIVATE) pr.emplace_back((size_t) rb.row0, (size_t) rb.row0 + rb.n_rows);
        std::sort(pr.begin(), pr.end());
        for (const auto &r : pr) {
            if (!m->private_rows.empty() && m->private_rows.back().second == r.first) m->private_rows.back().second = r.second;
            else m->private_rows.push_back(r);
        }
        m->n_private_rb = pr.size();
        size_t covered = 0;
        for (const auto &r : m->private_rows) covered += r.second - r.first;
        if (m->private_rows.size() > 4 || covered * 4 < nrows) m->private_rows.clear();
        m->use_private = !m->private_rows.empty();
        for (const SpxRowBlock &rb : s.rbs) m->max_slot_groups = std::max<size_t>(m->max_slot_groups, (rb.n_slots + 7u) / 8u);
    }
    {
        const size_t n = s.rbs.size();
        std::vector<uint64_t> upto(n + 1, 0);
        for (size_t i = 0; i < n; ++i) {
            const uint64_t end = i + 1 < n ? s.rbs[i + 1].val_off : (uint64_t) s.values.size();
            upto[i + 1] = upto[i] + (end > s.rbs[i].val_off ? end - s.rbs[i].val_off : 0) + 64u + 2u * s.rbs[i].n_rows;
        }
        m->rb_upto = upto;
        m->rb_row0.resize(n);
        for (size_t i = 0; i < n; ++i) m->rb_row0[i] = s.rbs[i].row0;
        std::vector<size_t> starts(1, 0);
        for (size_t i = 1; i < n; ++i)
            if (s.rbs[i].flags & SPX_RB_PHASE_START) starts.push_back(i);
        starts.push_back(n);
        m->accum = n > 0 && (s.rbs[0].flags & SPX_RB_ACCUM) != 0;
        const size_t K = starts.size() - 1;
        if (m->accum && (K == 2 || K == 4 || K == 8)) {
            XcdSplit xs;
            const uint32_t per = (uint32_t)(8 / K);
            for (size_t k = 0; k < K; ++k) {
                const size_t lo = starts[k], hi = starts[k + 1];
                for (uint32_t j = 0; j < per; ++j) {
                    const uint64_t want = upto[lo] + (upto[hi] - upto[lo]) * j / per;
                    size_t i = (size_t)(std::lower_bound(upto.begin() + lo, upto.begin() + hi + 1, want) - upto.begin());
                    xs.first[k * per + j] = (uint32_t) std::min(std::max(i, lo), hi);
                }
            }
            xs.first[8] = (uint32_t) n;
            uint32_t longest = 0;
            for (uint32_t x = 0; x < 8; ++x) longest = std::max(longest, xs.first[x + 1] - xs.first[x]);
            m->xcd_split.push_back(xs);
            m->xcd_longest.push_back(longest);
            starts.assign(1, n);
        } else if (m->accum) {
            throw FatalError("column slices for one launch: 2, 4 or 8 of them");
        }
        for (size_t ph = 0; ph + 1 < starts.size(); ++ph) {
            const size_t lo = starts[ph], hi = starts[ph + 1];
            XcdSplit xs;
            xs.first[0] = (uint32_t) lo;
            for (uint32_t x = 1; x < 8; ++x) {
                const uint64_t want = upto[lo] + (upto[hi] - upto[lo]) * x / 8;
                size_t i = (size_t)(std::lower_bound(upto.begin() + lo, upto.begin() + hi + 1, want) - upto.begin());
                i = std::min(std::max<size_t>(i, xs.first[x - 1]), hi);
                xs.first[x] = (uint32_t) i;
            }
            xs.first[8] = (uint32_t) hi;
            uint32_t longest = 0;
            for (uint32_t x = 0; x < 8; ++x) longest = std::max(longest, xs.first[x + 1] - xs.first[x]);
            m->xcd_split.push_back(xs);
            m->xcd_longest.push_back(longest);
        }
    }
    {
        std::vector<uint32_t> order;
        if (s.band_order) {
            order.resize(s.rbs.size());
            for (size_t i = 0; i < order.size(); ++i) order[i] = (uint32_t) i;
            bool any = false;
            for (const XcdSplit &xs : m->xcd_split) {
                for (uint32_t x = 0; x < 8; ++x) {
                    size_t S = 0;
                    const std::vector<uint32_t> part = stream_band_order(s, xs.first[x], xs.first[x + 1], S);
                    if (part.empty()) continue;
                    std::copy(part.begin(), part.end(), order.begin() + xs.first[x]);
                    m->band_stride = S;
                    any = true;
                }
            }
            if (!any) order.clear();
        }
        if (order.empty()) {
            place.put(&m->values, s.values, 160);
            place.put(&m->descs, s.descs, 8);
            place.put(&m->rbs, s.rbs);
            place.put(&m->passes, s.passes, (size_t) s.pass_stride + 6 * MAX_WAVES_PER_BLOCK);
        } else {
            const size_t stride = s.pass_stride;
            std::vector<SpxRowBlock> &rbs = rbs_ordered;
            std::vector<SpxPass> &passes = passes_ordered;
            rbs.resize(s.rbs.size());
            passes.resize(s.passes.size());
            for (size_t i = 0; i < order.size(); ++i) {
                rbs[i] = s.rbs[order[i]];
                rbs[i].pass_off = (uint32_t)(i * stride);
                std::copy(s.passes.begin() + (size_t) order[i] * stride, s.passes.begin() + ((size_t) order[i] + 1) * stride,
                          passes.begin() + i * stride);
            }
            place.put(&m->values, s.values, 160);
            place.put(&m->descs, s.descs, 8);
            place.put(&m->rbs, rbs);
            place.put(&m->passes, passes, stride + 6 * MAX_WAVES_PER_BLOCK);
            m->launch_order.swap(order);
        }
    }
    if (m->has_symsegs && (size_t) m->lds_doubles * sizeof(double) + 8192u > 64u * 1024u) {
        spmv_allow_lds(SpmvFamily::symseg, 160u * 1024u);
        spmv_allow_lds(SpmvFamily::symseg_notile, 160u * 1024u);
    }
    if (s.deterministic) device_set_deterministic(m, true);
    else if (s.wave_tiles) device_set_wave_tiles(m, true);
    m->n_values = s.values.size(); m->n_descs = s.descs.size(); m->n_passes = s.passes.size();
    m->n_cidx = s.cidx.size(); m->n_segrows = s.segrows.size();
    m->value_bytes = s.values.size() * sizeof(double);
    m->index_bytes = s.index_bytes();
    try {
        place.flush(m, s.arena);
    } catch (...) {
        device_free(m);
        throw;
    }
    m->xw_budget = s.xw_budget;
    m->xw_gap = s.xw_gap;
    if (s.xw_budget && !symmetric && !m->accum && m->xcd_split.size() == 1 && !s.rbs.empty()) {
        try {
            XwPlan plan;
            plan_unit_xwindows(s, ncols, s.xw_budget, s.xw_gap, plan, host_threads());
            if (!m->launch_order.empty()) {
                const size_t stride = s.pass_stride;
                std::vector<SpxPass> po(plan.passes.size());
                std::vector<XwEntry> to(plan.tab.size());
                for (size_t i = 0; i < m->launch_order.size(); ++i) {
                    const size_t from = m->launch_order[i];
                    std::copy(plan.passes.begin() + from * stride, plan.passes.begin() + (from + 1) * stride, po.begin() + i * stride);
                    std::copy(plan.tab.begin() + from * XW_TAB, plan.tab.begin() + (from + 1) * XW_TAB, to.begin() + i * XW_TAB);
                }
                plan.passes.swap(po);
                plan.tab.swap(to);
            }
            if (plan.n_rb_windows && (size_t) plan.lds_doubles * sizeof(double) > 160u * 1024u) {
                log_msg(LOG_INFO, "unit windows: %u KB of LDS per workgroup do not fit, not used\n",
                        (unsigned) ((size_t) plan.lds_doubles * sizeof(double) / 1024u));
            } else if (plan.n_rb_windows) {
                auto up = [&](auto **dst, const auto &v, size_t slack) {
                    typedef typename std::remove_reference<decltype(v[0])>::type T;
                    const size_t bytes = (v.size() + slack) * sizeof(T);
                    HIP_CHECK(hipMalloc(reinterpret_cast<void **>(dst), bytes));
                    HIP_CHECK(hipMemset(*dst, 0, bytes));
                    HIP_CHECK(hipMemcpy(*dst, v.data(), v.size() * sizeof(T), hipMemcpyHostToDevice));
                };
                up(&m->passes_xw, plan.passes, (size_t) s.pass_stride + 6 * MAX_WAVES_PER_BLOCK);
                up(&m->xdescs, plan.xdescs, 8);
                up(&m->xw_tab, plan.tab, 0);
                m->lds_doubles_xw = plan.lds_doubles;
                m->xw_elems = plan.unit_elems_lds;
                m->xw_unit_elems = plan.unit_elems;
                m->xw_staged = plan.staged_doubles;
                m->xw_rowblocks = plan.n_rb_windows;
                m->xw_on = s.xw_on;
                if ((size_t) m->lds_doubles_xw * sizeof(double) > 64u * 1024u) spmv_xw_allow_lds(160u * 1024u);
                log_msg(LOG_INFO, "unit windows: %zu of %zu row-blocks, %.1f %% of the unit nonzeros read x from LDS, "
                        "%.2f doubles staged per such nonzero, %u KB of LDS per workgroup\n", plan.n_rb_windows, plan.n_rb_units,
                        100.0 * (double) plan.unit_elems_lds / (double) std::max<uint64_t>(plan.unit_elems, 1),
                        (double) plan.staged_doubles / (double) std::max<uint64_t>(plan.unit_elems_lds, 1),
                        (unsigned) (m->lds_doubles_xw * sizeof(double) / 1024u));
            }
        } catch (...) {
            device_free(m);
            throw;
        }
    }
    if (symmetric && s.sx_plan && m->has_symsegs && !m->has_symtiles &&
        m->xcd_split.size() == 1 && !s.rbs.empty() && !s.deterministic && !s.wave_tiles) {
        try {
            SxPlan plan;
            plan_sym_pipeline(s, plan, host_threads());
            const size_t lds_need = (size_t) m->lds_doubles * sizeof(double) + m->max_slot_groups * sizeof(uint32_t) +
                                    spmv_sx_header_bytes(s.pass_stride);
            if (!m->launch_order.empty()) {
                const size_t stride = s.pass_stride;
                std::vector<SpxPass> po(plan.passes.size());
                std::vector<uint32_t> no(plan.n_sx.size());
                for (size_t i = 0; i < m->launch_order.size(); ++i) {
                    std::copy(plan.passes.begin() + (size_t) m->launch_order[i] * stride,
                              plan.passes.begin() + ((size_t) m->launch_order[i] + 1) * stride, po.begin() + i * stride);
                    no[i] = plan.n_sx[m->launch_order[i]];
                }
                plan.passes.swap(po);
                plan.n_sx.swap(no);
            }
            if (plan.n_rb_sx && lds_need <= 160u * 1024u) {
                const size_t pbytes = (plan.passes.size() + (size_t) s.pass_stride + 6 * MAX_WAVES_PER_BLOCK) * sizeof(SpxPass);
                HIP_CHECK(hipMalloc(reinterpret_cast<void **>(&m->passes_sx), pbytes));
                HIP_CHECK(hipMemset(m->passes_sx, 0, pbytes));
                HIP_CHECK(hipMemcpy(m->passes_sx, plan.passes.data(), plan.passes.size() * sizeof(SpxPass), hipMemcpyHostToDevice));
                HIP_CHECK(hipMalloc(reinterpret_cast<void **>(&m->sx_tab), plan.n_sx.size() * sizeof(uint32_t)));
                HIP_CHECK(hipMemcpy(m->sx_tab, plan.n_sx.data(), plan.n_sx.size() * sizeof(uint32_t), hipMemcpyHostToDevice));
                m->sx_elems = plan.sx_elems;
                m->sx_sym_elems = plan.sym_elems;
                m->sx_rowblocks = plan.n_rb_sx;
                m->sx_on = s.sx_on;
                if (lds_need > 64u * 1024u) spmv_sx_allow_lds(160u * 1024u);
                log_msg(LOG_INFO, "read-once pipeline: %zu row-blocks, %llu of %llu read-once passes (%.1f %% of their nonzeros) "
                        "carry their geometry in the header\n", plan.n_rb_sx, (unsigned long long) plan.sx_passes,
                        (unsigned long long) plan.sym_passes,
                        100.0 * (double) plan.sx_elems / (double) std::max<uint64_t>(plan.sym_elems, 1));
            }
        } catch (...) {
            device_free(m);
            throw;
        }
    }
    if (!m->accum && !m->n_shared && m->xcd_split.size() == 1 && m->launch_order.empty() &&
        (!symmetric || !m->n_mirror_rows) && m->n_rb >= 64 &&
        m->nrows * sizeof(double) >= host_parts_min_bytes()) {
        try {
            m->xneed_piece = host_xpiece_doubles(m->ncols);
            stream_rowblock_xpieces(s, m->ncols, m->xneed_piece, m->rb_xneed, host_threads());
        } catch (...) {
            device_free(m);
            throw;
        }
    }
    return m;
}

void device_free(DeviceMatrix *m)
{
    if (!m) return;
    if (m->arena) {
        (void) hipFree(m->arena);
    } else {
        (void) hipFree(m->rbs); (void) hipFree(m->values); (void) hipFree(m->descs);
        (void) hipFree(m->passes);
        (void) hipFree(m->cidx); (void) hipFree(m->segrows); (void) hipFree(m->shared);
        (void) hipFree(m->carry);
        if (m->carry_mv) (void) hipFree(m->carry_mv);
        if (m->dvalues) (void) hipFree(m->dvalues);
        if (m->spill) (void) hipFree(m->spill);
        if (m->fix_ptr) (void) hipFree(m->fix_ptr);
        if (m->fix_idx) (void) hipFree(m->fix_idx);
        if (m->slot_col) (void) hipFree(m->slot_col);
        if (m->mirror_rows) (void) hipFree(m->mirror_rows);
        if (m->mirror_ptr) (void) hipFree(m->mirror_ptr);
        if (m->mirror_col) (void) hipFree(m->mirror_col);
        if (m->mirror_val) (void) hipFree(m->mirror_val);
    }
    if (m->passes_sx) (void) hipFree(m->passes_sx);
    if (m->sx_tab) (void) hipFree(m->sx_tab);
    if (m->passes_xw) (void) hipFree(m->passes_xw);
    if (m->xdescs) (void) hipFree(m->xdescs);
    if (m->xw_tab) (void) hipFree(m->xw_tab);
    if (m->d_x) (void) hipFree(m->d_x);
    if (m->d_y) (void) hipFree(m->d_y);
    if (m->p_x) (void) hipHostFree(m->p_x);
    if (m->p_y) (void) hipHostFree(m->p_y);
    if (m->host_stream) (void) hipStreamDestroy(m->host_stream);
    if (m->copy_stream) (void) hipStreamDestroy(m->copy_stream);
    if (m->up_stream) (void) hipStreamDestroy(m->up_stream);
    for (hipEvent_t e : m->stage_events) (void) hipEventDestroy(e);
    for (hipEvent_t e : m->part_events) (void) hipEventDestroy(e);
    delete m;
}

struct SpmvPart {
    XcdSplit split;
    uint32_t longest;
    bool first, last;
};
static void device_product(DeviceMatrix *m, int K, double alpha, const double *X, size_t ldx, double beta, double *Y,
                           size_t ldy, void *stream_, const SpmvPart *part);

void device_spmv(DeviceMatrix *m, double alpha, const double *d_x, double beta,
                 double *d_y, void *stream_)
{
    device_product(m, 1, alpha, d_x, 0, beta, d_y, 0, stream_, nullptr);
}

static bool diagonal_at_writeout(const DeviceMatrix *m) { return m->sym_fused && !m->sym_atomic; }

static KernelArgs kernel_args(const DeviceMatrix *m, double alpha, const double *d_x, double beta, double *d_y)
{
    KernelArgs a{};
    a.rbs = m->rbs; a.values = m->values; a.descs = m->descs; a.passes = m->passes;
    a.cidx = m->cidx; a.segrows = m->segrows;
    a.x = d_x; a.y = d_y; a.pass_stride = m->pass_stride;
    a.carry = m->carry; a.alpha = alpha; a.beta = beta; a.n_rb = m->n_rb;
    a.dvalues = diagonal_at_writeout(m) ? m->dvalues : nullptr;
    a.slot_col = m->slot_col;
    a.spill = m->spill;
    return a;
}

static bool launch_rowblocks(const DeviceMatrix *m, const KernelArgs &a, const XcdSplit &xcd_now, uint32_t blocks,
                             void *stream)
{
    if (!blocks) return false;
    const size_t lds = m->lds_doubles * sizeof(double);
    if (m->wave_tiles && !m->accum) {
        launch_spmv(m->has_tiles ? SpmvFamily::symtile_det : SpmvFamily::det, m->waves, blocks, (size_t) m->waves * lds,
                    stream, a, xcd_now);
        return m->has_tiles && m->n_spill != 0;
    }
    if (m->has_tiles) {
        const size_t lds_a = lds + m->max_slot_groups * sizeof(uint32_t);
        if (m->sym_atomic && m->has_symsegs && !m->has_symtiles && m->sx_on && m->passes_sx) {
            KernelArgs as = a;
            as.passes = m->passes_sx;
            launch_spmv_sx(m->waves, blocks, lds_a + spmv_sx_header_bytes(m->pass_stride), stream, as, xcd_now, m->sx_tab);
        } else if (m->sym_atomic && m->has_symsegs && !m->has_symtiles) {
            launch_spmv(SpmvFamily::symseg_notile, m->waves, blocks, lds_a, stream, a, xcd_now);
        } else if (m->sym_atomic && m->has_symsegs) {
            launch_spmv(SpmvFamily::symseg, m->waves, blocks, lds_a, stream, a, xcd_now);
        } else if (m->sym_atomic) {
            launch_spmv(SpmvFamily::symtile_atomic, m->waves, blocks, lds_a, stream, a, xcd_now);
        } else {
            launch_spmv(SpmvFamily::symtile, m->waves, blocks, lds, stream, a, xcd_now);
        }
        return m->n_spill && !m->sym_atomic;
    }
    if (m->accum) {
        launch_spmv(SpmvFamily::accum, m->waves, blocks, lds, stream, a, xcd_now);
    } else if (m->xw_on && m->passes_xw) {
        KernelArgs ax = a;
        ax.passes = m->passes_xw;
        ax.descs = m->xdescs;
        ax.xw_tab = m->xw_tab;
        launch_spmv_xw(m->waves, blocks, (size_t) m->lds_doubles_xw * sizeof(double), stream, ax, xcd_now);
    } else {
        launch_spmv(SpmvFamily::plain, m->waves, blocks, lds, stream, a, xcd_now);
    }
    return false;
}


static size_t mv_copies(const DeviceMatrix *m) { return m->wave_tiles && !m->accum ? (size_t) m->waves : 1u; }

static size_t mv_lds_bytes(const DeviceMatrix *m, int K, bool stage)
{
    return ((size_t) K * (mv_copies(m) * m->mv_rows + (stage ? m->mv_xwin : 0u))) * sizeof(double);
}

int device_mv_group(const DeviceMatrix *m)
{
    if (m->has_tiles || !m->carry_mv) return 1;
    for (int K = MV_MAX_GROUP; K >= 2; K /= 2)
        if (mv_lds_bytes(m, K, false) <= MV_LDS_BUDGET) return K;
    return 1;
}

static uint32_t mv_n_carry(const DeviceMatrix *m) { return m->n_carry ? m->n_carry : 1u; }

static void launch_rowblocks_mv(const DeviceMatrix *m, int K, const KernelArgs &a, size_t ldx, size_t ldy,
                                const XcdSplit &xcd_now, uint32_t blocks, void *stream)
{
    if (!blocks) return;
    MvArgs mv{};
    static_cast<StreamArgs &>(mv) = a;
    mv.x = a.x; mv.y = a.y; mv.ldx = ldx; mv.ldy = ldy;
    mv.carry = m->carry_mv; mv.n_carry = mv_n_carry(m);
    mv.dvalues = a.dvalues; mv.alpha = a.alpha; mv.beta = a.beta; mv.pass_stride = a.pass_stride;
    mv.stage = m->mv_xwin && mv_lds_bytes(m, K, true) <= MV_LDS_BUDGET ? 1u : 0u;
    const MvFamily family = m->wave_tiles && !m->accum ? MvFamily::det : m->accum ? MvFamily::accum : MvFamily::plain;
    launch_spmv_mv(family, K, m->waves, blocks, mv_lds_bytes(m, K, mv.stage != 0), stream, mv, xcd_now);
}

static void device_product(DeviceMatrix *m, int K, double alpha, const double *X, size_t ldx, double beta, double *Y,
                           size_t ldy, void *stream_, const SpmvPart *part)
{
    int cur = -1;
    if (hipGetDevice(&cur) != hipSuccess || cur != m->device)
        throw FatalError("the matrix lives on HIP device " + std::to_string(m->device) +
                         ", the calling thread's current device is " + std::to_string(cur));
    m->launched_since_edit = true;
    KernelArgs a = kernel_args(m, alpha, X, beta, Y);
    const bool fused = diagonal_at_writeout(m);

    const size_t n_launch = m->xcd_split.size();
    if (m->symmetric && !fused) {
        const size_t first = m->init_limited ? m->init_lo : 0, last = m->init_limited ? m->own_hi : m->nrows;
        auto init_rows = [&](size_t lo, size_t hi) {
            if (hi > lo && !abl::sym_no_init && (!part || part->first))
                launch_sym_init(stream_, K, Y, ldy, X, ldx, m->dvalues, lo, hi, m->own_lo, m->own_hi, alpha, beta);
        };
        if (K == 1 && m->sym_atomic && !m->wave_tiles && m->use_private && !abl::sym_no_private) {
            size_t at = first;
            for (const auto &r : m->private_rows) {
                if (r.second <= at) continue;
                if (r.first >= last) break;
                init_rows(at, std::min(std::max(r.first, at), last));
                at = std::max(at, r.second);
            }
            init_rows(at, last);
            a.dvalues_priv = m->dvalues;
            a.beta_priv = beta;
        }
        else
            init_rows(first, last);
        if (m->n_mirror_rows && (!part || part->first))
            launch_sym_mirror_rows(stream_, K, m->mirror_rows, m->mirror_ptr, m->mirror_col, m->mirror_val, X, ldx, Y, ldy,
                                   alpha, m->n_mirror_rows);
        a.beta = beta = 1.0;
    }
    if (m->accum && !m->symmetric) {
        const size_t lo = m->own_lo, hi = m->own_hi;
        if (hi > lo) launch_scale(stream_, K, Y, ldy, lo, hi, beta);
        a.beta = beta = 1.0;
    }
    bool need_symfix = false;
    for (size_t ph = 0; ph < n_launch; ++ph) {
        if (ph > 0) a.beta = 1.0;
        const XcdSplit &split = part ? part->split : m->xcd_split[ph];
        const uint32_t blocks = 8u * (part ? part->longest : m->xcd_longest[ph]);
        if (K == 1) need_symfix |= launch_rowblocks(m, a, split, blocks, stream_);
        else launch_rowblocks_mv(m, K, a, ldx, ldy, split, blocks, stream_);
    }
    if (part && !part->last) {
        HIP_CHECK(hipGetLastError());
        return;
    }
    if (m->n_shared)
        launch_fixup(stream_, K, m->shared, m->n_shared, K == 1 ? m->carry : m->carry_mv, mv_n_carry(m), Y, ldy, alpha,
                     beta, a.dvalues, X, ldx);
    if (need_symfix) launch_symfix(stream_, m->fix_ptr, m->fix_idx, m->spill, Y, alpha, m->nrows);
    HIP_CHECK(hipGetLastError());
}

void device_spmm(DeviceMatrix *m, double alpha, const double *X, size_t ldx, size_t nvec, double beta, double *Y,
                 size_t ldy, void *stream_)
{
    const int G = device_mv_group(m);
    for (size_t j = 0; j < nvec;) {
        int K = G;
        while (K > 1 && (size_t) K > nvec - j) K /= 2;
        device_product(m, K, alpha, X + j * ldx, ldx, beta, Y + j * ldy, ldy, stream_, nullptr);
        j += (size_t) K;
    }
}

size_t device_plan_chunks(DeviceMatrix *m, size_t K, std::vector<size_t> &row_bounds, int slot)
{
    DeviceMatrix::ChunkPlan &cp = m->chunks[slot < 0 || slot > 2 ? 0 : slot];
    if (K >= 2 && K == cp.asked && !cp.split.empty()) {
        row_bounds = cp.bounds;
        return cp.split.size();
    }
    row_bounds.clear();
    cp.split.clear();
    cp.longest.clear();
    cp.order.clear();
    cp.step_pieces.clear();
    cp.asked = K;
    const size_t n = m->n_rb;
    if (m->accum || m->n_shared || m->xcd_split.size() != 1 || !m->launch_order.empty() ||
        n < 64 || K < 2 || m->rb_upto.size() != n + 1)
        return 0;
    if (m->symmetric &&
        !(slot == 2 && m->sym_atomic && !m->wave_tiles && m->use_private && m->private_rows.size() == 1 &&
          !m->n_mirror_rows && !m->init_limited && m->own_lo == 0 && m->own_hi == m->nrows))
        return 0;
    for (size_t i = 1; i < n; ++i)
        if (m->rb_row0[i] < m->rb_row0[i - 1]) return 0;
    size_t base = 0;
    cp.front_longest = 0;
    if (m->symmetric) {
        const size_t p_lo = m->private_rows[0].first;
        const size_t i0 = (size_t) (std::lower_bound(m->rb_row0.begin(), m->rb_row0.end(), (uint32_t) p_lo) - m->rb_row0.begin());
        if (i0 >= n || m->rb_row0[i0] != p_lo || n - i0 != m->n_private_rb) return 0;
        base = i0;
    }
    K = std::min<size_t>(K, (n - base) / 32);
    if (K < 2) return 0;
    auto split_of = [&](size_t lo, size_t hi, uint32_t &longest) {
        XcdSplit xs;
        xs.first[0] = (uint32_t) lo;
        for (uint32_t x = 1; x < 8; ++x) {
            const uint64_t want = m->rb_upto[lo] + (m->rb_upto[hi] - m->rb_upto[lo]) * x / 8;
            size_t i = (size_t)(std::lower_bound(m->rb_upto.begin() + lo, m->rb_upto.begin() + hi + 1, want) - m->rb_upto.begin());
            xs.first[x] = (uint32_t) std::min(std::max<size_t>(i, xs.first[x - 1]), hi);
        }
        xs.first[8] = (uint32_t) hi;
        longest = 0;
        for (uint32_t x = 0; x < 8; ++x) longest = std::max(longest, xs.first[x + 1] - xs.first[x]);
        return xs;
    };
    if (base > 0) cp.front = split_of(0, base, cp.front_longest);
    std::vector<size_t> cut(K + 1, base);
    for (size_t k = 1; k < K; ++k) {
        const uint64_t want = m->rb_upto[base] + (m->rb_upto[n] - m->rb_upto[base]) * k / K;
        size_t i = (size_t)(std::lower_bound(m->rb_upto.begin(), m->rb_upto.end(), want) - m->rb_upto.begin());
        cut[k] = std::min(std::max(i, cut[k - 1]), n);
    }
    cut[K] = n;
    for (size_t k = 0; k < K; ++k) {
        const size_t lo = cut[k], hi = cut[k + 1];
        uint32_t longest = 0;
        cp.split.push_back(split_of(lo, hi, longest));
        cp.longest.push_back(longest);
        row_bounds.push_back(lo < n ? (size_t) m->rb_row0[lo] : m->own_hi);
    }
    if (m->symmetric)
        for (size_t &b : row_bounds) b = std::max(b, m->private_rows[0].first);
    if (m->symmetric) {
        row_bounds[0] = m->private_rows[0].first;
        row_bounds.push_back(m->private_rows[0].second);
    } else {
        row_bounds[0] = m->own_lo;
        row_bounds.push_back(m->own_hi);
    }
    cp.bounds = row_bounds;
    cp.order.clear();
    cp.step_pieces.clear();
    if (slot == 2 && m->rb_xneed.size() == n && m->xneed_piece) {
        const size_t P = (m->ncols + m->xneed_piece - 1) / m->xneed_piece;
        std::vector<uint64_t> need(K, 0ull);
        for (size_t k = 0; k < K; ++k)
            for (size_t i = cut[k]; i < cut[k + 1]; ++i) need[k] |= m->rb_xneed[i];
        uint64_t init_need = 0, front_need = 0;
        if (m->symmetric) {
            auto rows = [&](size_t lo, size_t hi) {
                for (size_t pc = lo / m->xneed_piece; hi > lo && pc <= (hi - 1) / m->xneed_piece && pc < P; ++pc) init_need |= 1ull << pc;
            };
            rows(0, m->private_rows[0].first);
            rows(m->private_rows[0].second, m->nrows);
            for (size_t i = 0; i < base; ++i) front_need |= m->rb_xneed[i];
        }
        uint64_t have = 0;
        std::vector<char> done(K, 0);
        for (size_t step = 0; step < K; ++step) {
            const uint64_t with = (step == 0 ? init_need : 0ull) | (step + 1 == K ? front_need : 0ull);
            size_t best = K;
            int best_new = 65;
            for (size_t k = 0; k < K; ++k) {
                const int fresh = __builtin_popcountll((need[k] | with) & ~have);
                if (!done[k] && fresh < best_new) { best_new = fresh; best = k; }
            }
            need[best] |= with;
// ... 226 lines not shown
        struct Piece { size_t lo, hi; };
        std::vector<Piece> pieces;
        std::vector<std::vector<size_t>> pieces_of(K);
        auto add_piece = [&](size_t lo, size_t hi, size_t part) {
            pieces_of[part].push_back(pieces.size());
            pieces.push_back(Piece{lo, hi});
        };
        for (size_t k = 0; k < K; ++k)
            if (bounds[k + 1] > bounds[k]) add_piece(bounds[k], bounds[k + 1], k);
        const size_t k_last = cp.order.size() == K ? cp.order[K - 1] : K - 1;
        const size_t n_own = pieces.size();
        if (bounds[0] > 0) add_piece(0, bounds[0], k_last);
        if (bounds[K] < m->nrows) add_piece(bounds[K], m->nrows, k_last);
        const size_t ev_piece = K, ev_up = K + pieces.size();
        while (m->part_events.size() < ev_up + K) {
            hipEvent_t e;
            HIP_CHECK(hipEventCreateWithFlags(&e, hipEventDisableTiming));
            m->part_events.push_back(e);
        }
        try {
            if (x_by_need) {
                m->x_version = 0;
            }
            for (size_t j = 0; j < K; ++j) {
                const size_t k = cp.order.size() == K ? cp.order[j] : j;
                if (x_by_need) {
                    for (uint32_t pc : cp.step_pieces[j]) {
                        const size_t off = (size_t) pc * m->xneed_piece * sizeof(double);
                        if (off >= xb) continue;
                        const size_t n = std::min(m->xneed_piece * sizeof(double), xb - off);
                        HIP_CHECK(hipMemcpyAsync(reinterpret_cast<char *>(m->d_x) + off, reinterpret_cast<const char *>(h_x) + off, n,
                                                 hipMemcpyHostToDevice, m->up_stream));
                    }
                    if (y_by_need) {
                        auto send_y = [&](const Piece &pc) {
                            const size_t off = pc.lo * sizeof(double), n = (pc.hi - pc.lo) * sizeof(double);
                            HIP_CHECK(hipMemcpyAsync(reinterpret_cast<char *>(m->d_y) + off, reinterpret_cast<const char *>(h_y) + off, n,
                                                     hipMemcpyHostToDevice, m->up_stream));
                        };
                        if (j == 0)
                            for (size_t i = n_own; i < pieces.size(); ++i) send_y(pieces[i]);
                        for (size_t i : pieces_of[k])
                            if (i < n_own) send_y(pieces[i]);
                    }
                    HIP_CHECK(hipEventRecord(m->part_events[ev_up + j], m->up_stream));
                    HIP_CHECK(hipStreamWaitEvent(st, m->part_events[ev_up + j], 0));
                }
                device_spmv_chunk(m, k, alpha, m->d_x, beta, m->d_y, st, 2, (j == 0 ? 1 : 0) | (j + 1 == K ? 2 : 0));
                HIP_CHECK(hipEventRecord(m->part_events[k], st));
                HIP_CHECK(hipStreamWaitEvent(m->copy_stream, m->part_events[k], 0));
                for (size_t i : pieces_of[k]) {
                    const size_t off = pieces[i].lo * sizeof(double), n = (pieces[i].hi - pieces[i].lo) * sizeof(double);
                    char *dst = reinterpret_cast<char *>(y_pinned ? h_y : m->p_y) + off;
                    HIP_CHECK(hipMemcpyAsync(dst, reinterpret_cast<char *>(m->d_y) + off, n, hipMemcpyDeviceToHost, m->copy_stream));
                    if (!y_pinned) HIP_CHECK(hipEventRecord(m->part_events[ev_piece + i], m->copy_stream));
                }
            }
            if (y_pinned) {
                HIP_CHECK(hipStreamSynchronize(m->copy_stream));
            } else {
                for (size_t j = 0; j < K; ++j)
                    for (size_t i : pieces_of[cp.order.size() == K ? cp.order[j] : j]) {
                        const size_t off = pieces[i].lo * sizeof(double), n = (pieces[i].hi - pieces[i].lo) * sizeof(double);
                        HIP_CHECK(hipEventSynchronize(m->part_events[ev_piece + i]));
                        copy_threads(reinterpret_cast<char *>(h_y) + off, reinterpret_cast<char *>(m->p_y) + off, n);
                    }
            }
            if (m->up_stream) HIP_CHECK(hipStreamSynchronize(m->up_stream));
            HIP_CHECK(hipStreamSynchronize(st));
            if (x_by_need) m->x_version = x_version;
            return;
        } catch (...) {
            if (m->up_stream) (void) hipStreamSynchronize(m->up_stream);
            (void) hipStreamSynchronize(m->copy_stream);
            (void) hipStreamSynchronize(st);
            (void) hipGetLastError();
            m->host_parts = 0;
            m->host_x_by_need = false;
            if (x_by_need) m->x_version = 0;
            throw;
        }
    }
    m->host_parts = 0;
    device_spmv(m, alpha, m->d_x, beta, m->d_y, st);
    if (after) after(m->d_y, st);
    if (y_pinned) {
        HIP_CHECK(hipMemcpyAsync(h_y, m->d_y, yb, hipMemcpyDeviceToHost, st));
        HIP_CHECK(hipStreamSynchronize(st));
        return;
    }
    const size_t pieces = (yb + STAGE_PIECE - 1) / STAGE_PIECE;
    if (pieces <= 1) {
        HIP_CHECK(hipMemcpyAsync(m->p_y, m->d_y, yb, hipMemcpyDeviceToHost, st));
        HIP_CHECK(hipStreamSynchronize(st));
        std::memcpy(h_y, m->p_y, yb);
        return;
    }
    while (m->stage_events.size() < pieces) {
        hipEvent_t e;
        HIP_CHECK(hipEventCreateWithFlags(&e, hipEventDisableTiming));
        m->stage_events.push_back(e);
    }
    for (size_t k = 0; k < pieces; ++k) {
        const size_t off = k * STAGE_PIECE, n = std::min(STAGE_PIECE, yb - off);
        HIP_CHECK(hipMemcpyAsync(reinterpret_cast<char *>(m->p_y) + off, reinterpret_cast<char *>(m->d_y) + off, n,
                                 hipMemcpyDeviceToHost, st));
        HIP_CHECK(hipEventRecord(m->stage_events[k], st));
    }
    for (size_t k = 0; k < pieces; ++k) {
        const size_t off = k * STAGE_PIECE, n = std::min(STAGE_PIECE, yb - off);
        HIP_CHECK(hipEventSynchronize(m->stage_events[k]));
        copy_threads(reinterpret_cast<char *>(h_y) + off, reinterpret_cast<char *>(m->p_y) + off, n);
    }
}

bool device_stream_is_capturing(void *stream)
{
    hipStreamCaptureStatus st = hipStreamCaptureStatusNone;
    if (hipStreamIsCapturing(static_cast<hipStream_t>(stream), &st) != hipSuccess) {
        (void) hipGetLastError();
        return false;
    }
    return st != hipStreamCaptureStatusNone;
}

void *device_host_alloc(size_t bytes)
{
    if (device_count() <= 0) return nullptr;
    void *p = nullptr;
    if (hipHostMalloc(&p, bytes ? bytes : 8, hipHostMallocPortable) != hipSuccess) {
        (void) hipGetLastError();
        return nullptr;
    }
    return p;
}

void device_host_free(void *p)
{
    if (p) (void) hipHostFree(p);
}

size_t device_host_parts_min_bytes() { return host_parts_min_bytes(); }

int device_host_register(void *p, size_t bytes)
{
    if (!p || !bytes || device_count() <= 0) return 0;
    const hipError_t e = hipHostRegister(p, bytes, hipHostRegisterDefault);
    if (e == hipSuccess) return 1;
    (void) hipGetLastError();
    return e == hipErrorHostMemoryAlreadyRegistered ? 2 : 0;
}

void device_host_unregister(void *p)
{
    if (!p) return;
    if (hipHostUnregister(p) != hipSuccess) (void) hipGetLastError();
}

template <typename T, typename A>
static void download(std::vector<T, A> &v, const T *d, size_t n)
{
    v.resize(n);
    if (n) HIP_CHECK(hipMemcpy(v.data(), d, n * sizeof(T), hipMemcpyDeviceToHost));
}

void device_download(const DeviceMatrix *m, GpuStream &s)
{
    HIP_CHECK(hipSetDevice(m->device));
    download(s.rbs, m->rbs, m->n_rb);
    download(s.values, m->values, m->n_values);
    download(s.descs, m->descs, m->n_descs);
    download(s.passes, m->passes, m->n_passes);
    if (!m->launch_order.empty()) {
        const size_t stride = m->pass_stride;
        std::vector<SpxRowBlock> rbs(s.rbs.size());
        std::vector<SpxPass> passes(s.passes.size());
        for (size_t i = 0; i < m->launch_order.size(); ++i) {
            const size_t o = m->launch_order[i];
            rbs[o] = s.rbs[i];
            rbs[o].pass_off = (uint32_t)(o * stride);
            std::copy(s.passes.begin() + i * stride, s.passes.begin() + (i + 1) * stride, passes.begin() + o * stride);
        }
        s.rbs.swap(rbs);
        s.passes.swap(passes);
    }
    download(s.cidx, m->cidx, m->n_cidx);
    download(s.segrows, m->segrows, m->n_segrows);
    download(s.shared, m->shared, m->n_shared);
    s.n_carry = m->n_carry;
    s.sym_fused = m->sym_fused;
    s.pass_stride = m->pass_stride;
    s.waves = (uint32_t) m->waves;
    s.n_spill = m->n_spill;
    s.lds_doubles = m->lds_doubles;
    if (m->n_mirror_rows) {
        download(s.mirror_rows, m->mirror_rows, m->n_mirror_rows);
        download(s.mirror_ptr, m->mirror_ptr, (size_t) m->n_mirror_rows + 1);
        download(s.mirror_col, m->mirror_col, m->n_mirror_nnz);
        download(s.mirror_val, m->mirror_val, m->n_mirror_nnz);
    }
    s.sym_atomic = m->sym_atomic;
    s.deterministic = m->deterministic;
    s.wave_tiles = m->wave_tiles;
    s.xw_on = device_get_xw(m);
    s.sx_plan = m->passes_sx != nullptr;
    s.sx_on = device_get_sx(m);
    s.xw_budget = m->xw_budget;
    s.xw_gap = m->xw_gap;
    if (m->n_spill) download(s.slot_group_col, m->slot_col, m->n_slot_col);
    if (m->n_spill) {
        download(s.fix_ptr, m->fix_ptr, m->n_fix_ptr);
        download(s.fix_idx, m->fix_idx, m->n_fix_idx);
    }
    if (m->symmetric) download(s.dvalues, m->dvalues, m->nrows);
}

static void quiesce_before_edit(DeviceMatrix *m)
{
    if (!m->launched_since_edit) return;
    const hipError_t e = hipDeviceSynchronize();
    if (e != hipSuccess) {
        (void) hipGetLastError();
        throw FatalError(std::string("cannot change a value while the device cannot be waited for (") + hipGetErrorString(e) +
                         "): is a stream being captured?");
    }
    m->launched_since_edit = false;
}

void device_poke_mirror(DeviceMatrix *m, size_t index, double value)
{
    if (index >= m->n_mirror_nnz) throw FatalError("value index outside the mirror list");
    HIP_CHECK(hipSetDevice(m->device));
    quiesce_before_edit(m);
    HIP_CHECK(hipMemcpy(m->mirror_val + index, &value, sizeof(value), hipMemcpyHostToDevice));
}

double device_peek(const DeviceMatrix *m, bool diagonal, size_t index)
{
    if (diagonal ? (!m->dvalues || index >= m->nrows) : index >= m->n_values)
        throw FatalError("value index outside the stream");
    HIP_CHECK(hipSetDevice(m->device));
    double v = 0.0;
    HIP_CHECK(hipMemcpy(&v, (diagonal ? m->dvalues : m->values) + index, sizeof(v), hipMemcpyDeviceToHost));
    return v;
}

void device_poke(DeviceMatrix *m, bool diagonal, size_t index, double value)
{
    if (diagonal ? (!m->dvalues || index >= m->nrows) : index >= m->n_values)
        throw FatalError("value index outside the stream");
    HIP_CHECK(hipSetDevice(m->device));
    quiesce_before_edit(m);
    HIP_CHECK(hipMemcpy((diagonal ? m->dvalues : m->values) + index, &value, sizeof(value),
                        hipMemcpyHostToDevice));
}

void device_info(const DeviceMatrix *m, DeviceMatrixInfo &info)
{
    info.n_rowblocks = m->n_rb;
    info.n_shared_rows = m->n_shared;
    info.value_bytes = m->value_bytes;
    info.index_bytes = m->index_bytes;
    info.device = m->device;
}

}
```

sparsex_amd/csrc/gpu_emit.hpp:

```cpp
#pragma once

#include "gpu_format.h"
#include "partition.hpp"

#include <utility>
#include <vector>

namespace spx {

struct SymTile {
    idx_t row0, col0;
    val_t v[64];
};

struct SymSeg {
    idx_t row, col;
    uint8_t width;
    val_t v[8];
};
typedef std::vector<SymSeg, BigAlloc<SymSeg>> SymSegVec;

struct GpuStream {
    ValVec values;
    std::vector<SpxUnitDesc> descs;
    std::vector<SpxPass> passes;
    std::vector<uint8_t> cidx;
    std::vector<uint16_t> segrows;
    std::vector<SpxRowBlock> rbs;
    std::vector<SpxSharedRow> shared;
    uint32_t n_carry = 0;
    std::vector<val_t> dvalues;
    bool sym_fused = false;
    std::vector<uint32_t> spill_col;
    std::vector<uint32_t> fix_ptr, fix_idx;
    std::vector<uint32_t> slot_group_col;
    std::vector<std::pair<uint32_t, uint32_t>> direct_cols;
    std::vector<uint32_t> mirror_rows;
    std::vector<uint32_t> mirror_ptr;
    std::vector<uint32_t> mirror_col;
    std::vector<val_t> mirror_val;
    bool sym_atomic = false;
    bool deterministic = false;
    bool wave_tiles = false;
    uint32_t n_spill = 0;
    uint32_t lds_doubles = SPX_MAX_RB_ROWS;
    uint32_t pass_stride = 0;
    uint32_t waves = 4;
    bool band_order = false;
    bool arena = false;
    uint32_t xw_budget = 0, xw_gap = 16;
    bool xw_on = false;
    bool sx_plan = false, sx_on = false;
    size_t nnz_stored = 0;
    size_t n_unit_elems = 0;
    size_t n_delta_elems = 0;
    size_t n_units = 0;

    size_t n_pass_used() const
    {
        size_t n = 0;
        for (const SpxRowBlock &rb : rbs) n += rb.n_pass;
        return n;
    }
    size_t index_bytes() const
    {
        return descs.size() * sizeof(SpxUnitDesc) + n_pass_used() * sizeof(SpxPass) + cidx.size() +
               (sym_atomic ? slot_group_col.size() : fix_ptr.size() + fix_idx.size()) * 4 +
               (mirror_rows.size() + mirror_ptr.size() + mirror_col.size()) * 4 +
               segrows.size() * 2 + rbs.size() * sizeof(SpxRowBlock);
    }
};

struct GpuEmitParams {
    size_t target_elems = 2048;
    size_t max_rows = SPX_MAX_RB_ROWS;
    size_t sym_min_run = 2;
    size_t sym_max_run = SPX_MAX_SEG_WIDTH;
    size_t wide_rows = SPX_MAX_RB_ROWS;
    bool skip_empty = false;
    bool stack_segments = true;
    bool recut_linear = true;
    bool inline_desc = true;
    bool keep_units = true;
    bool sym_remine = true;
    bool x_window = true;
    int sym_segments = -1;
    bool sym_pure_passes = true;
    bool sym_once = true;
    const std::vector<SymTile> *tiles = nullptr;
    const SymSegVec *symsegs = nullptr;
};

void emit_gpu(const Partition &p, const GpuEmitParams &prm, GpuStream &out, unsigned nthreads = 1);

void append_stream(GpuStream &dst, GpuStream &&src, uint64_t values_placed_at = UINT64_MAX);

void finalize_stream(GpuStream &s, size_t nrows);

void mark_private_rowblocks(GpuStream &s, size_t nrows, idx_t own_lo, idx_t own_hi);

void append_sym_expanded(const Partition &lower, Partition &out, bool remine_upper = true);

struct SymRange { idx_t lo, hi; };
struct MirrorPoint { idx_t row, col; val_t val; };
void build_sym_ranges(const std::vector<Partition> &lowers, const std::vector<SymRange> &ranges,
                      bool want_tiles, std::vector<Partition> &outs,
                      std::vector<std::vector<SymTile>> &tiles, unsigned nthreads,
                      std::vector<MirrorPoint> *sparse_mirror = nullptr,
                      std::vector<SymSegVec> *symsegs = nullptr, size_t min_run = 2, size_t max_run = SPX_MAX_SEG_WIDTH);

inline void unit_elem_coords(const Elem &u, size_t k, idx_t &r, idx_t &c)
{
    const idx_t d = (idx_t) u.delta;
    switch (u.type) {
    case ENC_H:  r = u.row;               c = u.col + (idx_t) k * d; return;
    case ENC_V:  r = u.row + (idx_t) k * d; c = u.col;               return;
    case ENC_D:  r = u.row + (idx_t) k * d; c = u.col + (idx_t) k * d; return;
    case ENC_AD: r = u.row + (idx_t) k * d; c = u.col - (idx_t) k * d; return;
    default: break;
    }
    const idx_t a = (idx_t) enc_block_align(u.type);
    if (enc_is_block_row(u.type)) {
        r = u.row + (idx_t) k % a;
        c = u.col + (idx_t) k / a;
    } else {
        r = u.row + (idx_t) k / a;
        c = u.col + (idx_t) k % a;
    }
}

}
// ... 1 lines not shown
```

sparsex_amd/csrc/handles.hpp:

```cpp
#pragma once

#include <sparsex/sparsex.h>
#include <sparsex_hip.h>

#include "csx_emit.hpp"
#include "device.hpp"
#include "gpu_emit.hpp"
#include "input.hpp"
#include "xwindows.hpp"
#include "sxplan.hpp"

#include <algorithm>
#include <functional>
#include <memory>
#include <mutex>
#include <string>
#include <vector>
#include <thread>

namespace spx { struct DistPlan; }

using namespace spx;

struct input {
    spx_index_t nrows, ncols, nnz;
    char type;
    MatrixInput *mat;
};

struct partition {
    size_t nr_partitions;
    size_t *parts;
    int *nodes;
    int *affinity;
    spx_index_t *row_start;
    spx_index_t *row_end;
};

struct matrix {
    spx_index_t nrows = 0, ncols = 0, nnz = 0;
    int symmetric = 0;
    spx_perm_t *permutation = SPX_INVALID_PERM;
    size_t nr_partitions = 0;
    size_t first_part = 0, last_part = 0;
    std::vector<PartBounds> bounds;
    std::vector<Partition> parts;
    std::vector<std::thread> release_threads;
    template <class F> void release_later(F &&f)
    {
        std::function<void()> work(std::forward<F>(f));
        try {
            release_threads.emplace_back([work] { work(); });
        } catch (const std::exception &) {
            work();
        }
    }
    void release_wait()
    {
        for (std::thread &t : release_threads)
            if (t.joinable()) t.join();
        release_threads.clear();
    }
    ~matrix() { release_wait(); }
    std::vector<std::vector<val_t>> diag;
    std::vector<std::unique_ptr<CsxStream>> exported;
    std::vector<std::vector<spx_index_t>> exported_rows_info;
    bool full_colind = false;
    DeviceMatrix *dev = nullptr;
    std::unique_ptr<GpuStream> host_stream;
    std::unique_ptr<GpuStream> index;
    idx_t own_lo = 0, own_hi = 0;
    std::vector<idx_t> conflict_rows;
    std::vector<idx_t> halo_cols;
    idx_t first_block_row = 0;
    spx::DistPlan *dist = nullptr;
    GpuEmitParams emit_params;
    bool auto_rb = false;
    double rb_scale = 1.0;
    int waves = 4;
    size_t col_phases = 1;
    bool col_concurrent = false;
    bool host_only = false;
    bool has_tiles = false;
    bool sym_atomic = false;
    bool deterministic = false;
    bool has_symtiles = false;
    bool has_symsegs = false;
    int spill_mode = -1;
    int wave_tiles = -1;
    int unit_windows = -1;
    bool xw_on = false;
    bool rb_joined = false;
    int sym_pipeline = -1;
    bool sx_on = false;
    uint32_t xw_budget = 3072, xw_gap = 16;
    std::unique_ptr<spx::XwPlan> xw_inspect;
    std::unique_ptr<spx::SxPlan> sx_inspect;
    int device_ordinal = -1;
    std::vector<std::vector<idx_t>> spans;
    std::vector<idx_t> max_span;
    size_t nnz_stored = 0, n_unit_elems = 0, n_delta_elems = 0, n_units = 0;
    size_t value_bytes = 0, index_bytes = 0, n_rowblocks = 0, n_shared = 0;
    double tune_seconds = 0.0, emit_seconds = 0.0;
    std::string log;
    std::mutex mtx;
};

inline idx_t dist_first_init_row(const matrix &A)
{
    idx_t first = A.first_block_row;
    if (A.conflict_rows.empty()) return first;
    if (A.has_tiles) first = std::min(first, A.conflict_rows.front());
    return std::max(first, std::min(A.conflict_rows.front(), A.own_lo));
}
```

sparsex_amd/csrc/stream_index.cpp:

```cpp
#include "stream_index.hpp"

#include "threads.hpp"

#include <algorithm>
#include <cstdlib>
#include <cstring>

namespace spx {

namespace {

inline uint32_t popcount_upto(uint64_t mask, uint32_t lane)
{
    const uint64_t m = lane >= 63 ? mask : (mask & ((2ull << lane) - 1ull));
    return (uint32_t) __builtin_popcountll(m);
}

struct LaneSeg { int64_t row; int64_t col0; int64_t dcol_elem; bool ok; };

inline void unit_lane(const GpuStream &s, const SpxRowBlock &rb, const SpxPass &ps, uint32_t l,
                      int64_t &row, int64_t &col, uint32_t *slot = nullptr)
{
    const uint32_t stride = ps.kind == SPX_PASS_SYMSEG ? 2u : 1u;
    const uint32_t rank = (uint32_t) ps.rank0 + stride * popcount_upto(spx_pass_mask(&ps), l);
// ... 168 lines not shown
    const size_t n = s.rbs.size();
    mask.assign(n, 0ull);
    if (!piece || piece * 64 < ncols) throw FatalError("pieces of x: more than 64");
    const int64_t last = ncols ? (int64_t) ncols - 1 : 0;
    constexpr size_t CHUNK = 64;
    parallel_for((n + CHUNK - 1) / CHUNK, nthreads, [&](size_t c) {
        for (size_t i = c * CHUNK; i < std::min(n, (c + 1) * CHUNK); ++i) {
            const SpxRowBlock &rb = s.rbs[i];
            uint64_t m = 0;
            auto hit = [&](int64_t c0, int64_t c1) {
                c0 = std::min(std::max<int64_t>(c0, 0), last);
                c1 = std::min(std::max<int64_t>(c1, 0), last);
                for (size_t p = (size_t) c0 / piece; p <= (size_t) c1 / piece; ++p) m |= 1ull << p;
            };
            if (rb.xwin_len) hit((int64_t) rb.xwin_base, (int64_t) rb.xwin_base + rb.xwin_len - 1);
            for (uint32_t t = 0; t < rb.n_pass; ++t) {
                const SpxPass &ps = s.passes[(size_t) rb.pass_off + t];
                const uint32_t nseg = ps.nseg, W = ps.width;
                if (ps.kind == SPX_PASS_GATHER_LDS || nseg == 0) continue;
                if (is_gather(ps)) {
                    for (uint32_t l = 0; l < nseg; ++l)
                        for (uint32_t w = 0; w < W; ++w) {
                            const int64_t col = gather_col(s, rb, ps, (size_t) ps.elem0 + l + (size_t) w * nseg);
                            hit(col, col);
                        }
                } else if (ps.kind == SPX_PASS_SYMTILE) {
                    for (uint32_t l = 0; l < nseg; l += 8) {
                        const SpxUnitDesc &d = s.descs[(size_t) rb.desc_off + ps.rank0 + (l >> 3)];
                        hit((int64_t) d.col0, (int64_t) d.col0 + 7);
                    }
                } else {
                    const uint64_t starts = spx_pass_mask(&ps);
                    uint32_t first = 0;
                    for (uint32_t l = 1; l <= nseg; ++l) {
                        if (l < nseg && !((starts >> l) & 1ull)) continue;
                        int64_t r, ca, cb;
                        unit_lane(s, rb, ps, first, r, ca);
                        unit_lane(s, rb, ps, l - 1, r, cb);
                        hit(std::min(ca, cb), std::max(ca, cb) + (int64_t) W);
                        first = l;
                    }
                }
            }
            if (rb.n_rows && !s.dvalues.empty()) hit((int64_t) rb.row0, (int64_t) rb.row0 + rb.n_rows - 1);
            mask[i] = m;
        }
    });
    for (uint32_t c : s.mirror_col)
        if (!mask.empty()) mask[0] |= 1ull << ((size_t) std::min<int64_t>((int64_t) c, last) / piece);
}

void stream_locate_mirror(const GpuStream &s, idx_t row, idx_t col, std::vector<size_t> &out)
{
    auto it = std::lower_bound(s.mirror_rows.begin(), s.mirror_rows.end(), (uint32_t) row);
    if (it == s.mirror_rows.end() || *it != (uint32_t) row) return;
    const size_t t = (size_t) (it - s.mirror_rows.begin());
    for (uint32_t k = s.mirror_ptr[t]; k < s.mirror_ptr[t + 1]; ++k)
        if (s.mirror_col[k] == (uint32_t) col) out.push_back(k);
}

namespace {

void band_offsets(const GpuStream &s, const SpxRowBlock &rb, int64_t gap, std::vector<int64_t> &out)
{
    std::vector<int64_t> cols;
    for (uint32_t t = 0; t < rb.n_pass; ++t) {
        const SpxPass &ps = s.passes[(size_t) rb.pass_off + t];
        if (ps.kind != SPX_PASS_UNIT && ps.kind != SPX_PASS_SYMSEG) continue;
        const uint32_t stride = ps.kind == SPX_PASS_SYMSEG ? 2u : 1u;
        const uint32_t n = popcount_upto(spx_pass_mask(&ps), (uint32_t) ps.nseg - 1u) + 1u;
        for (uint32_t k = 0; k < n; ++k)
            cols.push_back((int64_t) s.descs[(size_t) rb.desc_off + ps.rank0 + stride * k].col0);
    }
    out.clear();
    if (cols.empty()) return;
    std::sort(cols.begin(), cols.end());
    out.push_back(cols[0] - (int64_t) rb.row0);
    for (size_t i = 1; i < cols.size(); ++i)
        if (cols[i] - cols[i - 1] > gap) out.push_back(cols[i] - (int64_t) rb.row0);
}

}

std::vector<uint32_t> stream_band_order(const GpuStream &s, size_t lo, size_t hi, size_t &stride_rows)
{
    stride_rows = 0;
    std::vector<uint32_t> order;
    if (hi <= lo + 512) return order;
    std::vector<int64_t> found, off;
    const size_t samples = 48;
    for (size_t k = 0; k < samples; ++k) {
        const SpxRowBlock &rb = s.rbs[lo + (hi - lo) * (2 * k + 1) / (2 * samples)];
        const int64_t rows = std::max<int64_t>(rb.n_rows, 64);
        band_offsets(s, rb, 4 * rows, off);
        for (size_t i = 0; i + 2 < off.size() && off.size() <= 8; ++i) {
            const int64_t d1 = off[i + 1] - off[i], d2 = off[i + 2] - off[i + 1];
            if (d1 < 32 * rows || std::llabs(d1 - d2) > 8) continue;
            found.push_back((d1 + d2) / 2);
            break;
        }
    }
    if (found.size() * 4 < samples * 3) return order;
    std::sort(found.begin(), found.end());
    const int64_t S = found[found.size() / 2];
    size_t agree = 0;
    for (int64_t v : found) agree += std::llabs(v - S) <= 8 ? 1 : 0;
    if (agree * 4 < samples * 3 || S <= 0) return order;
    const int64_t row_first = (int64_t) s.rbs[lo].row0;
    int64_t rows_total = 0;
    for (size_t i = lo; i < hi; ++i) {
        if ((int64_t) s.rbs[i].row0 < row_first) return std::vector<uint32_t>();
        rows_total += s.rbs[i].n_rows;
    }
    if ((int64_t) s.rbs[hi - 1].row0 - row_first < 3 * S) return order;
    const int64_t avg_rows = std::max<int64_t>(rows_total / (int64_t)(hi - lo), 1);
    const int64_t strip = std::max<int64_t>(24 * avg_rows, 1);
    struct Key { int64_t strip, plane, pos; uint32_t idx; };
    std::vector<Key> keys(hi - lo);
    for (size_t i = lo; i < hi; ++i) {
        const int64_t r = (int64_t) s.rbs[i].row0 - row_first;
        keys[i - lo] = Key{(r % S) / strip, r / S, r % S, (uint32_t) i};
    }
    std::sort(keys.begin(), keys.end(), [](const Key &a, const Key &b) {
        if (a.strip != b.strip) return a.strip < b.strip;
        if (a.plane != b.plane) return a.plane < b.plane;
        return a.pos < b.pos;
    });
    order.resize(hi - lo);
    for (size_t k = 0; k < keys.size(); ++k) order[k] = keys[k].idx;
    stride_rows = (size_t) S;
    return order;
}

bool stream_validate(const GpuStream &s, size_t nrows, size_t ncols, size_t n_values,
                     std::string &why)
{
#define SPX_REQUIRE(cond, msg)                                                                   \
    do {                                                                                         \
        if (!(cond)) {                                                                           \
            why = msg;                                                                           \
            return false;                                                                        \
        }                                                                                        \
    } while (0)
    SPX_REQUIRE(s.rbs.empty() || s.pass_stride >= 1, "pass stride missing");
    SPX_REQUIRE(s.passes.size() == s.rbs.size() * (size_t) s.pass_stride, "pass table size");
    SPX_REQUIRE(s.waves == 2 || s.waves == 4 || s.waves == 8, "wavefronts per workgroup");
    {
        size_t n_accum = 0, n_phase = 0;
        for (size_t i = 0; i < s.rbs.size(); ++i) {
            n_accum += (s.rbs[i].flags & SPX_RB_ACCUM) ? 1 : 0;
            n_phase += (i && (s.rbs[i].flags & SPX_RB_PHASE_START)) ? 1 : 0;
        }
        SPX_REQUIRE(n_accum == 0 || n_accum == s.rbs.size(), "column-slice flag on some row-blocks only");
        SPX_REQUIRE(n_accum == 0 || n_phase == 1 || n_phase == 3 || n_phase == 7, "column slices in one launch: 2, 4 or 8");
        bool any_private = false;
        for (const SpxRowBlock &rb : s.rbs) any_private = any_private || (rb.flags & SPX_RB_PRIVATE);
        if (any_private) {
            std::vector<char> reached(nrows, 0);
            for (uint32_t c : s.slot_group_col)
                for (size_t k = 0; k < 8; ++k)
                    if ((size_t) c + k < nrows) reached[(size_t) c + k] = 1;
            for (uint32_t r : s.mirror_rows)
                if (r < nrows) reached[r] = 1;
            for (const SpxRowBlock &rb : s.rbs) {
                SPX_REQUIRE((size_t) rb.pass_off + rb.n_pass <= s.passes.size(), "pass range");
                for (uint32_t t = 0; t < rb.n_pass; ++t) {
                    const SpxPass &ps = s.passes[(size_t) rb.pass_off + t];
                    if (ps.kind != SPX_PASS_SYMSEG) continue;
                    for (uint32_t l = 0; l < ps.nseg; ++l) {
                        const uint32_t rank = (uint32_t) ps.rank0 + 2u * popcount_upto(spx_pass_mask(&ps), l);
                        SPX_REQUIRE((size_t) rb.desc_off + rank + 1 < s.descs.size(), "descriptor range");
                        int64_t r, c;
                        uint32_t slot;
                        unit_lane(s, rb, ps, l, r, c, &slot);
                        if (slot != SPX_NO_SLOT) continue;
                        for (uint32_t w = 0; w < ps.width; ++w)
                            if (c + w >= 0 && (size_t)(c + w) < nrows) reached[(size_t)(c + w)] = 1;
                    }
                }
            }
            for (const SpxRowBlock &rb : s.rbs) {
                if (!(rb.flags & SPX_RB_PRIVATE)) continue;
                SPX_REQUIRE(!(rb.flags & SPX_RB_SHARED), "a row-block that stores its rows holds part of an over-long row");
                for (uint32_t r = 0; r < rb.n_rows; ++r)
                    SPX_REQUIRE((size_t) rb.row0 + r < nrows && !reached[(size_t) rb.row0 + r],
                                "a row-block that stores its rows is added to by another one");
            }
        }
    }
    SPX_REQUIRE(s.lds_doubles <= SPX_MAX_WIDE_SLOTS + SPX_MAX_WIDE_ROWS + SPX_MAX_XWIN, "LDS budget");
    SPX_REQUIRE(s.n_spill == 0 || (s.fix_ptr.size() == nrows + 1 && s.fix_idx.size() == s.n_spill),
                "spill lists");
    for (size_t i = 0; i + 1 < s.fix_ptr.size(); ++i)
        SPX_REQUIRE(s.fix_ptr[i] <= s.fix_ptr[i + 1], "spill list order");
    SPX_REQUIRE(s.fix_ptr.empty() || s.fix_ptr.back() == s.fix_idx.size(), "spill list end");
    for (uint32_t k : s.fix_idx) SPX_REQUIRE(k < s.n_spill, "spill index");
    for (uint32_t c : s.spill_col) SPX_REQUIRE(c < nrows, "spill columns");
    SPX_REQUIRE(s.mirror_rows.empty() ? s.mirror_ptr.size() <= 1 && s.mirror_col.empty()
                                      : s.mirror_ptr.size() == s.mirror_rows.size() + 1 &&
                                        s.mirror_ptr.back() == s.mirror_col.size(), "mirror list sizes");
    SPX_REQUIRE(s.mirror_val.empty() || s.mirror_val.size() == s.mirror_col.size(), "mirror list values");
    for (size_t i = 0; i < s.mirror_rows.size(); ++i)
        SPX_REQUIRE(s.mirror_rows[i] < nrows && s.mirror_ptr[i] <= s.mirror_ptr[i + 1] &&
                    (i == 0 || s.mirror_rows[i] > s.mirror_rows[i - 1]), "mirror list rows");
    for (uint32_t c : s.mirror_col) SPX_REQUIRE(c < ncols, "mirror list column");
    SPX_REQUIRE(s.slot_group_col.size() * 8 == s.n_spill, "slot groups");
    for (uint32_t c : s.slot_group_col) SPX_REQUIRE(c % 8 == 0 && (size_t) c + 8 <= nrows, "slot group column");
    SPX_REQUIRE(s.dvalues.empty() || s.dvalues.size() == nrows, "diagonal length");
    bool tiles = false;
    for (size_t i = 0; i < s.rbs.size(); ++i) {
        const SpxRowBlock &rb = s.rbs[i];
        SPX_REQUIRE(rb.n_rows >= 1 && rb.n_rows <= SPX_MAX_WIDE_ROWS, "row-block rows");
        SPX_REQUIRE((size_t) rb.row0 + rb.n_rows <= nrows, "row-block row range");
        SPX_REQUIRE(rb.pass_off == i * (size_t) s.pass_stride && rb.n_pass <= s.pass_stride,
// ... 85 lines not shown
```

sparsex_amd/csrc/stream_index.hpp:

```cpp
#pragma once

#include "gpu_emit.hpp"

#include <string>
#include <vector>

namespace spx {

void stream_locate(const GpuStream &s, idx_t row, idx_t col, std::vector<size_t> &out);

void stream_locate_mirror(const GpuStream &s, idx_t row, idx_t col, std::vector<size_t> &out);

void stream_touched_rows(const GpuStream &s, idx_t below, std::vector<idx_t> &rows);

void stream_read_cols(const GpuStream &s, idx_t own_lo, idx_t own_hi, size_t ncols, std::vector<idx_t> &cols);

void stream_rowblock_xpieces(const GpuStream &s, size_t ncols, size_t piece, std::vector<uint64_t> &mask, unsigned nthreads);

std::vector<uint32_t> stream_band_order(const GpuStream &s, size_t lo, size_t hi, size_t &stride_rows);

bool stream_validate(const GpuStream &s, size_t nrows, size_t ncols, size_t n_values,
                     std::string &why);

}
```

Before: 1231.

## Replace band ordering with autotuned XCD sweep order of row-blocks

```diff
diff --git a/include/sparsex_hip.h b/include/sparsex_hip.h
--- a/include/sparsex_hip.h
+++ b/include/sparsex_hip.h
@@ -154,7 +154,7 @@
     int64_t unit_window_elems;
     int64_t unit_window_staged;
     int32_t sym_pipeline;
-    int32_t reserved0;
+    int32_t xcd_sweep;
     int64_t sym_pipeline_elems;
 } spx_hip_info_t;
 
@@ -188,6 +188,7 @@
 int spx_hip_mat_host_parts(const spx_matrix_t *A);
 int spx_hip_mat_host_order(const spx_matrix_t *A, int32_t *order, int cap);
 int64_t spx_hip_mat_x_pieces(spx_matrix_t *A, size_t piece, uint64_t *mask, uint32_t *row0, uint32_t *n_rows, size_t cap);
+int64_t spx_hip_mat_sweep_order(spx_matrix_t *A, uint32_t *order, size_t cap, uint32_t first[9], uint64_t meta[6]);
 
 typedef struct {
     const spx_value_t *values;
diff --git a/sparsex_amd/api.py b/sparsex_amd/api.py
--- a/sparsex_amd/api.py
+++ b/sparsex_amd/api.py
@@ -42,7 +42,7 @@
                 ("quad", C.c_int32), ("col_slices", C.c_int32),
                 ("unit_windows", C.c_int32), ("unit_window_lds", C.c_int32),
                 ("unit_window_elems", C.c_int64), ("unit_window_staged", C.c_int64),
-                ("sym_pipeline", C.c_int32), ("reserved0", C.c_int32), ("sym_pipeline_elems", C.c_int64)]
+                ("sym_pipeline", C.c_int32), ("xcd_sweep", C.c_int32), ("sym_pipeline_elems", C.c_int64)]
 
 
 class SxPlan(C.Structure):
@@ -299,6 +299,20 @@
             raise SpxError("spx_hip_mat_info failed")
         return inf
 
+    def sweep_order(self):
+        L = lib()
+        L.spx_hip_mat_sweep_order.restype = C.c_int64
+        L.spx_hip_mat_sweep_order.argtypes = [C.c_void_p, C.c_void_p, C.c_size_t, C.c_void_p, C.c_void_p]
+        n_rb = int(self.info().n_rowblocks)
+        order = np.zeros(max(n_rb, 1), dtype=np.uint32)
+        first = np.zeros(9, dtype=np.uint32)
+        meta = np.zeros(6, dtype=np.uint64)
+        n = L.spx_hip_mat_sweep_order(self.handle, order.ctypes.data, n_rb, first.ctypes.data, meta.ctypes.data)
+        if n < 0:
+            raise SpxError("spx_hip_mat_sweep_order failed")
+        return {"order": order[:n] if n else None, "first": first, "stride": int(meta[0]), "origin": int(meta[1]),
+                "lo": int(meta[2]), "hi": int(meta[3]), "heaviest": int(meta[4]), "heaviest_contiguous": int(meta[5])}
+
     def unit_windows(self, budget=4096, gap=16):
         pl = XwPlan()
         L = lib()
diff --git a/sparsex_amd/csrc/api.cpp b/sparsex_amd/csrc/api.cpp
--- a/sparsex_amd/csrc/api.cpp
+++ b/sparsex_amd/csrc/api.cpp
@@ -601,7 +601,7 @@
     if (sym) mark_private_rowblocks(gs, (size_t) A->nrows, A->own_lo, A->own_hi);
     std::vector<std::pair<uint32_t, uint32_t>>().swap(gs.direct_cols);
     gs.waves = (uint32_t) A->waves;
-    gs.band_order = Config::instance().get_bool("spx.gpu.band_order");
+    gs.xcd_sweep = A->sweep_on;
     gs.arena = Config::instance().get_bool("spx.gpu.arena");
     gs.xw_budget = (A->unit_windows != 0 && !A->deterministic && !sym) ? (A->rb_joined ? std::max(A->xw_budget, JOINED_XW_BUDGET) : A->xw_budget) : 0u;
     gs.xw_gap = A->xw_gap;
@@ -1002,6 +1002,13 @@
     }
     A->sym_pipeline = sx_mode == "auto" ? -1 : (sx_mode == "true" ? 1 : 0);
     A->sx_on = sx_mode == "true";
+    const std::string sw_mode = cfg.get_str("spx.gpu.xcd_sweep");
+    if (sw_mode != "auto" && sw_mode != "true" && sw_mode != "false") {
+        log_msg(LOG_ERR, "spx.gpu.xcd_sweep: true, false or auto\n");
+        throw FatalError("bad spx.gpu.xcd_sweep");
+    }
+    A->xcd_sweep = sym ? 0 : (sw_mode == "auto" ? -1 : (sw_mode == "true" ? 1 : 0));
+    A->sweep_on = A->xcd_sweep == 1;
     const std::string ph_mode = cfg.get_str("spx.gpu.col_phases");
     const bool ph_conc = ph_mode.size() == 2 && ph_mode[0] == 'c';
     long ph_fixed = ph_mode == "auto" ? 0 : strtol(ph_mode.c_str() + (ph_conc ? 1 : 0), nullptr, 10);
@@ -1039,6 +1046,21 @@
         A->sx_on = t1 < 0.985 * t0;
         device_set_sx(A->dev, A->sx_on);
         log_msg(LOG_INFO, "read-once pipeline: %s (%.2f us per SpMV with, %.2f without)\n", A->sx_on ? "on" : "off", 1e6 * t1, 1e6 * t0);
+    }
+    if (A->dev && A->xcd_sweep == -1 && device_has_sweep(A->dev) && A->nnz_stored >= 100000) {
+        A->release_wait();
+        const double t_est = device_time_spmv(A->dev, 2, 3);
+        const int N = (int) std::min(100.0, std::max(8.0, 0.02 / std::max(t_est, 1e-7)));
+        auto best_of = [&](bool on) {
+            device_set_sweep(A->dev, on);
+            double best = device_time_spmv(A->dev, std::max(2, N / 10), N);
+            for (int rep = 0; rep < 3; ++rep) best = std::min(best, device_time_spmv(A->dev, 0, N));
+            return best;
+        };
+        const double t0 = best_of(false), t1 = best_of(true);
+        A->sweep_on = t1 < 0.985 * t0;
+        device_set_sweep(A->dev, A->sweep_on);
+        log_msg(LOG_INFO, "xcd sweep: %s (%.2f us per SpMV with, %.2f without)\n", A->sweep_on ? "on" : "off", 1e6 * t1, 1e6 * t0);
     }
     const double t_auto_end = now_sec();
     if (A->dev && !sym && ph_mode == "auto" && A->n_shared == 0 && A->nnz_stored >= 100000 &&
@@ -1646,6 +1668,8 @@
     A->sym_pipeline = gs->sx_on ? 1 : 0;
     A->xw_budget = gs->xw_budget;
     A->xw_gap = gs->xw_gap;
+    A->xcd_sweep = !A->symmetric && Config::instance().get_str("spx.gpu.xcd_sweep") == "true" ? 1 : 0;
+    A->sweep_on = gs->xcd_sweep = A->xcd_sweep == 1;
     {
         size_t slices = 1;
         for (size_t i = 1; i < gs->rbs.size(); ++i) slices += (gs->rbs[i].flags & SPX_RB_PHASE_START) ? 1 : 0;
@@ -2086,6 +2110,23 @@
         if (n_rows) n_rows[i] = s->rbs[i].n_rows;
     }
     return (int64_t) m.size();
+} SPX_C_BOUNDARY(return -1;)
+
+int64_t spx_hip_mat_sweep_order(spx_matrix_t *A, uint32_t *order, size_t cap, uint32_t first[9], uint64_t meta[6])
+try {
+    if (!A) { SETERROR_1(SPX_ERR_ARG_INVALID, "invalid argument"); return -1; }
+    const GpuStream *s = A->host_stream ? A->host_stream.get() : A->index.get();
+    if (!s) { SETERROR_1(SPX_ERR_TUNED_MAT, "matrix holds no descriptor stream"); return -1; }
+    std::lock_guard<std::mutex> lk(A->mtx);
+    SweepOrder so;
+    const bool found = !A->symmetric && stream_sweep_order(*s, stream_work_prefix(*s, A->value_bytes / sizeof(val_t)), so);
+    if (first) std::copy(so.first, so.first + 9, first);
+    if (meta) {
+        meta[0] = so.stride_rows; meta[1] = so.origin_row; meta[2] = so.lo; meta[3] = so.hi;
+        meta[4] = so.heaviest; meta[5] = so.heaviest_contiguous;
+    }
+    for (size_t i = 0; order && i < so.order.size() && i < cap; ++i) order[i] = so.order[i];
+    return found ? (int64_t) so.order.size() : 0;
 } SPX_C_BOUNDARY(return -1;)
 
 spx_error_t spx_hip_mat_sym_pipeline(spx_matrix_t *A, spx_hip_sx_plan_t *out)
@@ -2177,6 +2218,7 @@
         info->sym_pipeline = device_get_sx(A->dev) ? 1 : 0;
         info->sym_pipeline_elems = (int64_t) esx;
     }
+    info->xcd_sweep = A->dev && device_get_sweep(A->dev) ? 1 : 0;
     info->tune_seconds = A->tune_seconds;
     info->emit_seconds = A->emit_seconds;
     return SPX_SUCCESS;
diff --git a/sparsex_amd/csrc/config.cpp b/sparsex_amd/csrc/config.cpp
--- a/sparsex_amd/csrc/config.cpp
+++ b/sparsex_amd/csrc/config.cpp
@@ -50,7 +50,7 @@
     props_["spx.gpu.waves"] = "0";
     props_["spx.gpu.inline_desc"] = "true";
     props_["spx.gpu.arena"] = "false";
-    props_["spx.gpu.band_order"] = "false";
+    props_["spx.gpu.xcd_sweep"] = "auto";
     props_["spx.gpu.col_phases"] = "auto";
     props_["spx.gpu.keep_units"] = "true";
     props_["spx.gpu.recut_linear"] = "true";
diff --git a/sparsex_amd/csrc/device.hpp b/sparsex_amd/csrc/device.hpp
--- a/sparsex_amd/csrc/device.hpp
+++ b/sparsex_amd/csrc/device.hpp
@@ -64,6 +64,10 @@
 void device_xw_info(const DeviceMatrix *m, uint64_t &elems_lds, uint64_t &unit_elems, uint64_t &staged_doubles,
                     uint32_t &lds_bytes);
 
+bool device_has_sweep(const DeviceMatrix *m);
+void device_set_sweep(DeviceMatrix *m, bool on);
+bool device_get_sweep(const DeviceMatrix *m);
+
 bool device_has_sx(const DeviceMatrix *m);
 void device_set_sx(DeviceMatrix *m, bool on);
 bool device_get_sx(const DeviceMatrix *m);
diff --git a/sparsex_amd/csrc/device_runtime.cpp b/sparsex_amd/csrc/device_runtime.cpp
--- a/sparsex_amd/csrc/device_runtime.cpp
+++ b/sparsex_amd/csrc/device_runtime.cpp
@@ -54,8 +54,14 @@
     std::vector<XcdSplit> xcd_split;
     std::vector<uint32_t> xcd_longest;
     bool accum = false;
-    std::vector<uint32_t> launch_order;
-    size_t band_stride = 0;
+    std::vector<uint32_t> sweep_order;
+    XcdSplit sweep_split{};
+    uint32_t sweep_longest = 0;
+    size_t sweep_stride = 0;
+    SpxRowBlock *rbs_sw = nullptr;
+    SpxPass *passes_sw = nullptr, *passes_xw_sw = nullptr;
+    XwEntry *xw_tab_sw = nullptr;
+    bool sweep_on = false;
     bool launched_since_edit = true;
     bool has_symsegs = false;
     bool has_symtiles = false;
@@ -219,8 +225,6 @@
     Placement place;
     const std::vector<double> no_doubles;
     std::vector<double> dv;
-    std::vector<SpxRowBlock> rbs_ordered;
-    std::vector<SpxPass> passes_ordered;
     place.put(&m->cidx, s.cidx, 64);
     place.put(&m->segrows, s.segrows, 80);
     place.put(&m->shared, s.shared);
@@ -286,11 +290,7 @@
     }
     {
         const size_t n = s.rbs.size();
-        std::vector<uint64_t> upto(n + 1, 0);
-        for (size_t i = 0; i < n; ++i) {
-            const uint64_t end = i + 1 < n ? s.rbs[i + 1].val_off : (uint64_t) s.values.size();
-            upto[i + 1] = upto[i] + (end > s.rbs[i].val_off ? end - s.rbs[i].val_off : 0) + 64u + 2u * s.rbs[i].n_rows;
-        }
+        const std::vector<uint64_t> upto = stream_work_prefix(s, s.values.size());
         m->rb_upto = upto;
         m->rb_row0.resize(n);
         for (size_t i = 0; i < n; ++i) m->rb_row0[i] = s.rbs[i].row0;
@@ -337,48 +337,10 @@
             m->xcd_longest.push_back(longest);
         }
     }
-    {
-        std::vector<uint32_t> order;
-        if (s.band_order) {
-            order.resize(s.rbs.size());
-            for (size_t i = 0; i < order.size(); ++i) order[i] = (uint32_t) i;
-            bool any = false;
-            for (const XcdSplit &xs : m->xcd_split) {
-                for (uint32_t x = 0; x < 8; ++x) {
-                    size_t S = 0;
-                    const std::vector<uint32_t> part = stream_band_order(s, xs.first[x], xs.first[x + 1], S);
-                    if (part.empty()) continue;
-                    std::copy(part.begin(), part.end(), order.begin() + xs.first[x]);
-                    m->band_stride = S;
-                    any = true;
-                }
-            }
-            if (!any) order.clear();
-        }
-        if (order.empty()) {
-            place.put(&m->values, s.values, 160);
-            place.put(&m->descs, s.descs, 8);
-            place.put(&m->rbs, s.rbs);
-            place.put(&m->passes, s.passes, (size_t) s.pass_stride + 6 * MAX_WAVES_PER_BLOCK);
-        } else {
-            const size_t stride = s.pass_stride;
-            std::vector<SpxRowBlock> &rbs = rbs_ordered;
-            std::vector<SpxPass> &passes = passes_ordered;
-            rbs.resize(s.rbs.size());
-            passes.resize(s.passes.size());
-            for (size_t i = 0; i < order.size(); ++i) {
-                rbs[i] = s.rbs[order[i]];
-                rbs[i].pass_off = (uint32_t)(i * stride);
-                std::copy(s.passes.begin() + (size_t) order[i] * stride, s.passes.begin() + ((size_t) order[i] + 1) * stride,
-                          passes.begin() + i * stride);
-            }
-            place.put(&m->values, s.values, 160);
-            place.put(&m->descs, s.descs, 8);
-            place.put(&m->rbs, rbs);
-            place.put(&m->passes, passes, stride + 6 * MAX_WAVES_PER_BLOCK);
-            m->launch_order.swap(order);
-        }
-    }
+    place.put(&m->values, s.values, 160);
+    place.put(&m->descs, s.descs, 8);
+    place.put(&m->rbs, s.rbs);
+    place.put(&m->passes, s.passes, (size_t) s.pass_stride + 6 * MAX_WAVES_PER_BLOCK);
     if (m->has_symsegs && (size_t) m->lds_doubles * sizeof(double) + 8192u > 64u * 1024u) {
         spmv_allow_lds(SpmvFamily::symseg, 160u * 1024u);
         spmv_allow_lds(SpmvFamily::symseg_notile, 160u * 1024u);
@@ -401,18 +363,6 @@
         try {
             XwPlan plan;
             plan_unit_xwindows(s, ncols, s.xw_budget, s.xw_gap, plan, host_threads());
-            if (!m->launch_order.empty()) {
-                const size_t stride = s.pass_stride;
-                std::vector<SpxPass> po(plan.passes.size());
-                std::vector<XwEntry> to(plan.tab.size());
-                for (size_t i = 0; i < m->launch_order.size(); ++i) {
-                    const size_t from = m->launch_order[i];
-                    std::copy(plan.passes.begin() + from * stride, plan.passes.begin() + (from + 1) * stride, po.begin() + i * stride);
-                    std::copy(plan.tab.begin() + from * XW_TAB, plan.tab.begin() + (from + 1) * XW_TAB, to.begin() + i * XW_TAB);
-                }
-                plan.passes.swap(po);
-                plan.tab.swap(to);
-            }
             if (plan.n_rb_windows && (size_t) plan.lds_doubles * sizeof(double) > 160u * 1024u) {
                 log_msg(LOG_INFO, "unit windows: %u KB of LDS per workgroup do not fit, not used\n",
                         (unsigned) ((size_t) plan.lds_doubles * sizeof(double) / 1024u));
@@ -452,18 +402,6 @@
             plan_sym_pipeline(s, plan, host_threads());
             const size_t lds_need = (size_t) m->lds_doubles * sizeof(double) + m->max_slot_groups * sizeof(uint32_t) +
                                     spmv_sx_header_bytes(s.pass_stride);
-            if (!m->launch_order.empty()) {
-                const size_t stride = s.pass_stride;
-                std::vector<SpxPass> po(plan.passes.size());
-                std::vector<uint32_t> no(plan.n_sx.size());
-                for (size_t i = 0; i < m->launch_order.size(); ++i) {
-                    std::copy(plan.passes.begin() + (size_t) m->launch_order[i] * stride,
-                              plan.passes.begin() + ((size_t) m->launch_order[i] + 1) * stride, po.begin() + i * stride);
-                    no[i] = plan.n_sx[m->launch_order[i]];
-                }
-                plan.passes.swap(po);
-                plan.n_sx.swap(no);
-            }
             if (plan.n_rb_sx && lds_need <= 160u * 1024u) {
                 const size_t pbytes = (plan.passes.size() + (size_t) s.pass_stride + 6 * MAX_WAVES_PER_BLOCK) * sizeof(SpxPass);
                 HIP_CHECK(hipMalloc(reinterpret_cast<void **>(&m->passes_sx), pbytes));
@@ -486,7 +424,7 @@
             throw;
         }
     }
-    if (!m->accum && !m->n_shared && m->xcd_split.size() == 1 && m->launch_order.empty() &&
+    if (!m->accum && !m->n_shared && m->xcd_split.size() == 1 &&
         (!symmetric || !m->n_mirror_rows) && m->n_rb >= 64 &&
         m->nrows * sizeof(double) >= host_parts_min_bytes()) {
         try {
@@ -497,7 +435,86 @@
             throw;
         }
     }
+    if (!symmetric && !m->accum && !m->has_tiles && m->xcd_split.size() == 1) {
+        try {
+            SweepOrder so;
+            const bool found = stream_sweep_order(s, m->rb_upto, so);
+            if (so.stride_rows)
+                log_msg(LOG_INFO, "xcd sweep: bands %zu rows apart, row-blocks [%zu, %zu) of %zu; heaviest list %.3f of the mean "
+                        "(contiguous parts: %.3f): %s\n", so.stride_rows, so.lo, so.hi, s.rbs.size(),
+                        8.0 * (double) so.heaviest / (double) std::max<uint64_t>(m->rb_upto.back(), 1),
+                        8.0 * (double) so.heaviest_contiguous / (double) std::max<uint64_t>(m->rb_upto.back(), 1),
+                        found ? "an order" : "no order");
+            if (found) {
+                m->sweep_order.swap(so.order);
+                std::copy(so.first, so.first + 9, m->sweep_split.first);
+                for (uint32_t x = 0; x < 8; ++x) m->sweep_longest = std::max(m->sweep_longest, so.first[x + 1] - so.first[x]);
+                m->sweep_stride = so.stride_rows;
+                if (s.xcd_sweep) device_set_sweep(m, true);
+            }
+        } catch (...) {
+            device_free(m);
+            throw;
+        }
+    }
     return m;
+}
+
+bool device_has_sweep(const DeviceMatrix *m) { return !m->sweep_order.empty(); }
+bool device_get_sweep(const DeviceMatrix *m) { return m->sweep_on && m->rbs_sw; }
+
+static void free_sweep(DeviceMatrix *m)
+{
+    if (m->rbs_sw) (void) hipFree(m->rbs_sw);
+    if (m->passes_sw) (void) hipFree(m->passes_sw);
+    if (m->passes_xw_sw) (void) hipFree(m->passes_xw_sw);
+    if (m->xw_tab_sw) (void) hipFree(m->xw_tab_sw);
+    m->rbs_sw = nullptr;
+    m->passes_sw = m->passes_xw_sw = nullptr;
+    m->xw_tab_sw = nullptr;
+}
+
+void device_set_sweep(DeviceMatrix *m, bool on)
+{
+    m->sweep_on = on && !m->sweep_order.empty();
+    HIP_CHECK(hipSetDevice(m->device));
+    if (!m->sweep_on) {
+        if (m->rbs_sw) {
+            HIP_CHECK(hipDeviceSynchronize());
+            free_sweep(m);
+        }
+        return;
+    }
+    if (m->rbs_sw) return;
+    const std::vector<uint32_t> &order = m->sweep_order;
+    const size_t n = order.size(), stride = m->pass_stride;
+    const size_t slack = stride + 6 * MAX_WAVES_PER_BLOCK;
+    auto permuted = [&](auto **dst, const auto *src, size_t per, size_t slack_elems, auto &&fix) {
+        typedef typename std::remove_cv<typename std::remove_reference<decltype(*src)>::type>::type T;
+        std::vector<T> from(n * per), to(n * per);
+        if (n * per != 0) HIP_CHECK(hipMemcpy(from.data(), src, n * per * sizeof(T), hipMemcpyDeviceToHost));
+        for (size_t i = 0; i < n; ++i) {
+            std::copy(from.begin() + (size_t) order[i] * per, from.begin() + ((size_t) order[i] + 1) * per, to.begin() + i * per);
+            fix(to[i * per], i);
+        }
+        const size_t bytes = (n * per + slack_elems) * sizeof(T);
+        HIP_CHECK(hipMalloc(reinterpret_cast<void **>(dst), bytes));
+        HIP_CHECK(hipMemset(*dst, 0, bytes));
+        if (n * per != 0) HIP_CHECK(hipMemcpy(*dst, to.data(), n * per * sizeof(T), hipMemcpyHostToDevice));
+    };
+    try {
+        if (m->n_passes != n * stride) throw FatalError("sweep order: the pass headers are not strided");
+        permuted(&m->rbs_sw, m->rbs, 1, 0, [&](SpxRowBlock &rb, size_t i) { rb.pass_off = (uint32_t) (i * stride); });
+        permuted(&m->passes_sw, m->passes, stride, slack, [](SpxPass &, size_t) {});
+        if (m->passes_xw) {
+            permuted(&m->passes_xw_sw, m->passes_xw, stride, slack, [](SpxPass &, size_t) {});
+            permuted(&m->xw_tab_sw, m->xw_tab, (size_t) XW_TAB, 0, [](XwEntry &, size_t) {});
+        }
+    } catch (...) {
+        free_sweep(m);
+        m->sweep_on = false;
+        throw;
+    }
 }
 
 void device_free(DeviceMatrix *m)
@@ -521,6 +538,7 @@
         if (m->mirror_col) (void) hipFree(m->mirror_col);
         if (m->mirror_val) (void) hipFree(m->mirror_val);
     }
+    free_sweep(m);
     if (m->passes_sx) (void) hipFree(m->passes_sx);
     if (m->sx_tab) (void) hipFree(m->sx_tab);
     if (m->passes_xw) (void) hipFree(m->passes_xw);
@@ -544,12 +562,12 @@
     bool first, last;
 };
 static void device_product(DeviceMatrix *m, int K, double alpha, const double *X, size_t ldx, double beta, double *Y,
-                           size_t ldy, void *stream_, const SpmvPart *part);
+                           size_t ldy, void *stream_, const SpmvPart *part, bool sweep = false);
 
 void device_spmv(DeviceMatrix *m, double alpha, const double *d_x, double beta,
                  double *d_y, void *stream_)
 {
-    device_product(m, 1, alpha, d_x, 0, beta, d_y, 0, stream_, nullptr);
+    device_product(m, 1, alpha, d_x, 0, beta, d_y, 0, stream_, nullptr, true);
 }
 
 static bool diagonal_at_writeout(const DeviceMatrix *m) { return m->sym_fused && !m->sym_atomic; }
@@ -568,7 +586,7 @@
 }
 
 static bool launch_rowblocks(const DeviceMatrix *m, const KernelArgs &a, const XcdSplit &xcd_now, uint32_t blocks,
-                             void *stream)
+                             void *stream, bool sweep = false)
 {
     if (!blocks) return false;
     const size_t lds = m->lds_doubles * sizeof(double);
@@ -598,9 +616,9 @@
         launch_spmv(SpmvFamily::accum, m->waves, blocks, lds, stream, a, xcd_now);
     } else if (m->xw_on && m->passes_xw) {
         KernelArgs ax = a;
-        ax.passes = m->passes_xw;
+        ax.passes = sweep ? m->passes_xw_sw : m->passes_xw;
         ax.descs = m->xdescs;
-        ax.xw_tab = m->xw_tab;
+        ax.xw_tab = sweep ? m->xw_tab_sw : m->xw_tab;
         launch_spmv_xw(m->waves, blocks, (size_t) m->lds_doubles_xw * sizeof(double), stream, ax, xcd_now);
     } else {
         launch_spmv(SpmvFamily::plain, m->waves, blocks, lds, stream, a, xcd_now);
@@ -641,7 +659,7 @@
 }
 
 static void device_product(DeviceMatrix *m, int K, double alpha, const double *X, size_t ldx, double beta, double *Y,
-                           size_t ldy, void *stream_, const SpmvPart *part)
+                           size_t ldy, void *stream_, const SpmvPart *part, bool sweep)
 {
     int cur = -1;
     if (hipGetDevice(&cur) != hipSuccess || cur != m->device)
@@ -650,6 +668,11 @@
     m->launched_since_edit = true;
     KernelArgs a = kernel_args(m, alpha, X, beta, Y);
     const bool fused = diagonal_at_writeout(m);
+    sweep = sweep && !part && K == 1 && m->sweep_on && m->rbs_sw && m->xcd_split.size() == 1;
+    if (sweep) {
+        a.rbs = m->rbs_sw;
+        a.passes = m->passes_sw;
+    }
 
     const size_t n_launch = m->xcd_split.size();
     if (m->symmetric && !fused) {
@@ -685,9 +708,9 @@
     bool need_symfix = false;
     for (size_t ph = 0; ph < n_launch; ++ph) {
         if (ph > 0) a.beta = 1.0;
-        const XcdSplit &split = part ? part->split : m->xcd_split[ph];
-        const uint32_t blocks = 8u * (part ? part->longest : m->xcd_longest[ph]);
-        if (K == 1) need_symfix |= launch_rowblocks(m, a, split, blocks, stream_);
+        const XcdSplit &split = part ? part->split : (sweep ? m->sweep_split : m->xcd_split[ph]);
+        const uint32_t blocks = 8u * (part ? part->longest : (sweep ? m->sweep_longest : m->xcd_longest[ph]));
+        if (K == 1) need_symfix |= launch_rowblocks(m, a, split, blocks, stream_, sweep);
         else launch_rowblocks_mv(m, K, a, ldx, ldy, split, blocks, stream_);
     }
     if (part && !part->last) {
@@ -727,7 +750,7 @@
     cp.step_pieces.clear();
     cp.asked = K;
     const size_t n = m->n_rb;
-    if (m->accum || m->n_shared || m->xcd_split.size() != 1 || !m->launch_order.empty() ||
+    if (m->accum || m->n_shared || m->xcd_split.size() != 1 ||
         n < 64 || K < 2 || m->rb_upto.size() != n + 1)
         return 0;
     if (m->symmetric &&
@@ -1120,7 +1143,7 @@
         }
     }
     m->host_parts = 0;
-    device_spmv(m, alpha, m->d_x, beta, m->d_y, st);
+    device_product(m, 1, alpha, m->d_x, 0, beta, m->d_y, 0, st, nullptr);
     if (after) after(m->d_y, st);
     if (y_pinned) {
         HIP_CHECK(hipMemcpyAsync(h_y, m->d_y, yb, hipMemcpyDeviceToHost, st));
@@ -1209,19 +1232,6 @@
     download(s.values, m->values, m->n_values);
     download(s.descs, m->descs, m->n_descs);
     download(s.passes, m->passes, m->n_passes);
-    if (!m->launch_order.empty()) {
-        const size_t stride = m->pass_stride;
-        std::vector<SpxRowBlock> rbs(s.rbs.size());
-        std::vector<SpxPass> passes(s.passes.size());
-        for (size_t i = 0; i < m->launch_order.size(); ++i) {
-            const size_t o = m->launch_order[i];
-            rbs[o] = s.rbs[i];
-            rbs[o].pass_off = (uint32_t)(o * stride);
-            std::copy(s.passes.begin() + i * stride, s.passes.begin() + (i + 1) * stride, passes.begin() + o * stride);
-        }
-        s.rbs.swap(rbs);
-        s.passes.swap(passes);
-    }
     download(s.cidx, m->cidx, m->n_cidx);
     download(s.segrows, m->segrows, m->n_segrows);
     download(s.shared, m->shared, m->n_shared);
diff --git a/sparsex_amd/csrc/gpu_emit.hpp b/sparsex_amd/csrc/gpu_emit.hpp
--- a/sparsex_amd/csrc/gpu_emit.hpp
+++ b/sparsex_amd/csrc/gpu_emit.hpp
@@ -46,7 +46,7 @@
     uint32_t lds_doubles = SPX_MAX_RB_ROWS;
     uint32_t pass_stride = 0;
     uint32_t waves = 4;
-    bool band_order = false;
+    bool xcd_sweep = false;
     bool arena = false;
     uint32_t xw_budget = 0, xw_gap = 16;
     bool xw_on = false;
diff --git a/sparsex_amd/csrc/handles.hpp b/sparsex_amd/csrc/handles.hpp
--- a/sparsex_amd/csrc/handles.hpp
+++ b/sparsex_amd/csrc/handles.hpp
@@ -92,6 +92,8 @@
     bool xw_on = false;
     bool rb_joined = false;
     int sym_pipeline = -1;
+    int xcd_sweep = -1;
+    bool sweep_on = false;
     bool sx_on = false;
     uint32_t xw_budget = 3072, xw_gap = 16;
     std::unique_ptr<spx::XwPlan> xw_inspect;
diff --git a/sparsex_amd/csrc/stream_index.cpp b/sparsex_amd/csrc/stream_index.cpp
--- a/sparsex_amd/csrc/stream_index.cpp
+++ b/sparsex_amd/csrc/stream_index.cpp
@@ -274,15 +274,55 @@
 
 }
 
-std::vector<uint32_t> stream_band_order(const GpuStream &s, size_t lo, size_t hi, size_t &stride_rows)
-{
-    stride_rows = 0;
-    std::vector<uint32_t> order;
-    if (hi <= lo + 512) return order;
+std::vector<uint64_t> stream_work_prefix(const GpuStream &s, size_t n_values)
+{
+    const size_t n = s.rbs.size();
+    std::vector<uint64_t> upto(n + 1, 0);
+    for (size_t i = 0; i < n; ++i) {
+        const uint64_t end = i + 1 < n ? s.rbs[i + 1].val_off : (uint64_t) n_values;
+        upto[i + 1] = upto[i] + (end > s.rbs[i].val_off ? end - s.rbs[i].val_off : 0) + 64u + 2u * s.rbs[i].n_rows;
+    }
+    return upto;
+}
+
+void stream_contiguous_split(const std::vector<uint64_t> &upto, size_t lo, size_t hi, uint32_t first[9])
+{
+    first[0] = (uint32_t) lo;
+    for (uint32_t x = 1; x < 8; ++x) {
+        const uint64_t want = upto[lo] + (upto[hi] - upto[lo]) * x / 8;
+        size_t i = (size_t)(std::lower_bound(upto.begin() + lo, upto.begin() + hi + 1, want) - upto.begin());
+        first[x] = (uint32_t) std::min(std::max<size_t>(i, first[x - 1]), hi);
+    }
+    first[8] = (uint32_t) hi;
+}
+
+namespace {
+
+bool has_bands(const GpuStream &s, const SpxRowBlock &rb, int64_t S, std::vector<int64_t> &off)
+{
+    const int64_t rows = std::max<int64_t>(rb.n_rows, 64);
+    band_offsets(s, rb, 4 * rows, off);
+    for (size_t i = 0; i + 2 < off.size() && off.size() <= 8; ++i)
+        if (std::llabs(off[i + 1] - off[i] - S) <= 8 && std::llabs(off[i + 2] - off[i + 1] - S) <= 8) return true;
+    return false;
+}
+
+}
+
+bool stream_sweep_order(const GpuStream &s, const std::vector<uint64_t> &upto, SweepOrder &out)
+{
+    out = SweepOrder();
+    const size_t n = s.rbs.size();
+    if (n <= 512 || upto.size() != n + 1) return false;
+    for (size_t i = 0; i < n; ++i) {
+        if (s.rbs[i].flags & SPX_RB_ACCUM) return false;
+        if (i && ((s.rbs[i].flags & SPX_RB_PHASE_START) || s.rbs[i].row0 < s.rbs[i - 1].row0)) return false;
+    }
+    if (!s.dvalues.empty() || !s.mirror_rows.empty()) return false;
     std::vector<int64_t> found, off;
     const size_t samples = 48;
     for (size_t k = 0; k < samples; ++k) {
-        const SpxRowBlock &rb = s.rbs[lo + (hi - lo) * (2 * k + 1) / (2 * samples)];
+        const SpxRowBlock &rb = s.rbs[n * (2 * k + 1) / (2 * samples)];
         const int64_t rows = std::max<int64_t>(rb.n_rows, 64);
         band_offsets(s, rb, 4 * rows, off);
         for (size_t i = 0; i + 2 < off.size() && off.size() <= 8; ++i) {
@@ -292,36 +332,89 @@
             break;
         }
     }
-    if (found.size() * 4 < samples * 3) return order;
+    if (found.size() * 4 < samples * 3) return false;
     std::sort(found.begin(), found.end());
     const int64_t S = found[found.size() / 2];
     size_t agree = 0;
     for (int64_t v : found) agree += std::llabs(v - S) <= 8 ? 1 : 0;
-    if (agree * 4 < samples * 3 || S <= 0) return order;
-    const int64_t row_first = (int64_t) s.rbs[lo].row0;
-    int64_t rows_total = 0;
-    for (size_t i = lo; i < hi; ++i) {
-        if ((int64_t) s.rbs[i].row0 < row_first) return std::vector<uint32_t>();
-        rows_total += s.rbs[i].n_rows;
-    }
-    if ((int64_t) s.rbs[hi - 1].row0 - row_first < 3 * S) return order;
-    const int64_t avg_rows = std::max<int64_t>(rows_total / (int64_t)(hi - lo), 1);
-    const int64_t strip = std::max<int64_t>(24 * avg_rows, 1);
-    struct Key { int64_t strip, plane, pos; uint32_t idx; };
-    std::vector<Key> keys(hi - lo);
-    for (size_t i = lo; i < hi; ++i) {
-        const int64_t r = (int64_t) s.rbs[i].row0 - row_first;
-        keys[i - lo] = Key{(r % S) / strip, r / S, r % S, (uint32_t) i};
-    }
-    std::sort(keys.begin(), keys.end(), [](const Key &a, const Key &b) {
-        if (a.strip != b.strip) return a.strip < b.strip;
-        if (a.plane != b.plane) return a.plane < b.plane;
-        return a.pos < b.pos;
-    });
-    order.resize(hi - lo);
-    for (size_t k = 0; k < keys.size(); ++k) order[k] = keys[k].idx;
-    stride_rows = (size_t) S;
-    return order;
+    if (agree * 4 < samples * 3 || S < 8) return false;
+    out.stride_rows = (size_t) S;
+    size_t lo = 0, hi = n;
+    while (lo < n && !has_bands(s, s.rbs[lo], S, off)) ++lo;
+    while (hi > lo && !has_bands(s, s.rbs[hi - 1], S, off)) --hi;
+    out.lo = lo;
+    out.hi = hi;
+    if (hi <= lo + 512) return false;
+    const int64_t row_lo = (int64_t) s.rbs[lo].row0;
+    out.origin_row = (size_t) row_lo;
+    if ((int64_t) s.rbs[hi - 1].row0 - row_lo < 3 * S) return false;
+    uint64_t max_rb = 0, heaviest_contig = 0;
+    for (size_t i = lo; i < hi; ++i) max_rb = std::max(max_rb, upto[i + 1] - upto[i]);
+    uint32_t contig[9];
+    stream_contiguous_split(upto, 0, n, contig);
+    for (uint32_t k = 0; k < 8; ++k) heaviest_contig = std::max(heaviest_contig, upto[contig[k + 1]] - upto[contig[k]]);
+    out.heaviest_contiguous = heaviest_contig;
+    struct Key { int64_t plane, pos; uint32_t idx; };
+    const size_t n_pool = lo + (n - hi);
+    auto pool_rb = [&](size_t j) { return j < lo ? j : hi + (j - lo); };
+    auto order_from = [&](int64_t origin, std::vector<uint32_t> &order, uint32_t first[9]) {
+        std::vector<Key> strips[8];
+        for (size_t i = lo; i < hi; ++i) {
+            const int64_t r = (int64_t) s.rbs[i].row0 - origin;
+            strips[(size_t) ((r % S) * 8 / S)].push_back(Key{r / S, r % S, (uint32_t) i});
+        }
+        for (auto &st : strips)
+            std::sort(st.begin(), st.end(), [](const Key &a, const Key &b) {
+                return a.plane != b.plane ? a.plane < b.plane : (a.pos != b.pos ? a.pos < b.pos : a.idx < b.idx);
+            });
+        uint64_t strip_work[8], need[8], need_total = 0;
+        const uint64_t mean = upto[n] / 8, pool = upto[lo] + (upto[n] - upto[hi]);
+        for (uint32_t k = 0; k < 8; ++k) {
+            strip_work[k] = 0;
+            for (const Key &key : strips[k]) strip_work[k] += upto[(size_t) key.idx + 1] - upto[key.idx];
+            need[k] = mean > strip_work[k] ? mean - strip_work[k] : 0;
+            need_total += need[k];
+        }
+        order.clear();
+        order.reserve(n);
+        uint64_t heaviest = 0, dealt = 0, want = 0;
+        size_t j = 0;
+        for (uint32_t k = 0; k < 8; ++k) {
+            first[k] = (uint32_t) order.size();
+            want += need_total > pool ? (uint64_t) ((double) need[k] * (double) pool / (double) need_total)
+                                      : need[k] + (pool - need_total) / 8;
+            uint64_t work = strip_work[k];
+            const size_t j0 = j;
+            while (j < n_pool && (k == 7 || dealt + (upto[pool_rb(j) + 1] - upto[pool_rb(j)]) / 2 < want)) {
+                dealt += upto[pool_rb(j) + 1] - upto[pool_rb(j)];
+                work += upto[pool_rb(j) + 1] - upto[pool_rb(j)];
+                ++j;
+            }
+            for (size_t q = j0; q < j && q < lo; ++q) order.push_back((uint32_t) q);
+            for (const Key &key : strips[k]) order.push_back(key.idx);
+            for (size_t q = std::max(j0, lo); q < j; ++q) order.push_back((uint32_t) pool_rb(q));
+            heaviest = std::max(heaviest, work);
+        }
+        first[8] = (uint32_t) n;
+        return heaviest;
+    };
+    std::vector<uint32_t> order, trial;
+    uint64_t heaviest = ~0ull;
+    for (int64_t shift = 0; shift < 16; ++shift) {
+        const int64_t origin = row_lo - shift * S / 128;
+        if (origin < 0) break;
+        uint32_t first[9];
+        const uint64_t h = order_from(origin, trial, first);
+        if (h >= heaviest) continue;
+        heaviest = h;
+        order.swap(trial);
+        std::copy(first, first + 9, out.first);
+        out.origin_row = (size_t) origin;
+    }
+    out.heaviest = heaviest;
+    if (heaviest > heaviest_contig + max_rb) return false;
+    out.order.swap(order);
+    return true;
 }
 
 bool stream_validate(const GpuStream &s, size_t nrows, size_t ncols, size_t n_values,
diff --git a/sparsex_amd/csrc/stream_index.hpp b/sparsex_amd/csrc/stream_index.hpp
--- a/sparsex_amd/csrc/stream_index.hpp
+++ b/sparsex_amd/csrc/stream_index.hpp
@@ -17,7 +17,17 @@
 
 void stream_rowblock_xpieces(const GpuStream &s, size_t ncols, size_t piece, std::vector<uint64_t> &mask, unsigned nthreads);
 
-std::vector<uint32_t> stream_band_order(const GpuStream &s, size_t lo, size_t hi, size_t &stride_rows);
+std::vector<uint64_t> stream_work_prefix(const GpuStream &s, size_t n_values);
+void stream_contiguous_split(const std::vector<uint64_t> &upto, size_t lo, size_t hi, uint32_t first[9]);
+
+struct SweepOrder {
+    std::vector<uint32_t> order;
+    uint32_t first[9] = {0, 0, 0, 0, 0, 0, 0, 0, 0};
+    size_t lo = 0, hi = 0;
+    size_t stride_rows = 0, origin_row = 0;
+    uint64_t heaviest = 0, heaviest_contiguous = 0;
+};
+bool stream_sweep_order(const GpuStream &s, const std::vector<uint64_t> &upto, SweepOrder &out);
 
 bool stream_validate(const GpuStream &s, size_t nrows, size_t ncols, size_t n_values,
                      std::string &why);
```

After: 1202. 2.3% lower.
